# nh13/DWGSIM

Hardware: AMD Instinct MI355X
Metric: M read-pairs/sec (2x150 bp PE) (higher is better)
Workload: dtype u8

## Files before the change

dwgsim_amd/csrc/dw_host.cpp:

```cpp
#include <hip/hip_runtime.h>
#include <math.h>
#include <stdio.h>
#include <stdlib.h>
#include <string.h>
#include <limits.h>
#include <ctype.h>
#include <stdarg.h>
#include <stdint.h>
#include <sys/mman.h>
#include <mutex>
#include <thread>
#include <string>
#include <vector>
#include <algorithm>
#include <array>
#include <stddef.h>
#include <type_traits>
#include "../../include/dwgsim_hip.h"
#include "dw_kernels.hpp"
#include "dw_launch.hpp"
#include "dw_mutin.hpp"
#include "dw_mem.hpp"

using namespace dw;

namespace {

struct HostIns { std::vector<int32_t> pos; std::vector<uint32_t> len, off; std::vector<uint8_t> bases; };

struct Member {
    std::string name;
    int64_t l = 0, l_place = 0;
    uint32_t contig_index = 0;
    int32_t start = 0;
    int32_t reg_off = 0, n_reg = 0;
    uint32_t name_off = 0; int32_t name_fixed_len = 0;
    ResolvedContig rc;
};

struct GroupMem {
    DevMem d_ref, d_cells[2], d_view[2];
    DevMem d_ins_pos[2], d_ins_len[2], d_ins_off[2], d_ins_bases[2];
    DevMem d_names, d_reg, d_seg;
    std::vector<uint8_t> h_names; std::vector<int32_t> h_reg, h_seg;
    DevMem d_summ[2], d_summ2[2];
    DevMem d_refview, d_refsumm, d_refsumm2, d_dirty;
    DevEvent ev_walk, ev_walk0;
    DevMem d_hap_text[2], d_hap_rec, d_hap_pool;
    DevMem d_hap_chain[2];
    DevMem d_depth_pos, d_depth_cnt;
    HostMem h_wc;
};

struct WalkCounters {
    uint64_t unused0[7];
    uint64_t n_cand;
    uint32_t max_del;
    struct { uint32_t entries, bases; } ins[2];
    uint32_t unused1;
    uint32_t slot_over;
    uint32_t n_cand_true;
    uint64_t mut_debug[2];
    uint64_t n_listed;
    uint64_t unused2;
};
static_assert(std::is_standard_layout<WalkCounters>::value && sizeof(WalkCounters) == 16 * 8, "the walk's counter block is 16 u64 words");
static_assert(offsetof(WalkCounters, n_cand) == 7 * 8 && offsetof(WalkCounters, max_del) == 8 * 8 && offsetof(WalkCounters, ins) == 8 * 8 + 4 && offsetof(WalkCounters, slot_over) == 8 * 8 + 6 * 4 &&
              offsetof(WalkCounters, n_cand_true) == 8 * 8 + 7 * 4 && offsetof(WalkCounters, mut_debug) == 12 * 8 && offsetof(WalkCounters, n_listed) == 14 * 8, "every counter at the word the kernels were given before the block had a type");
struct WcSpan { size_t off, bytes; };
#define WC_SPAN(first, last) WcSpan{offsetof(WalkCounters, first), offsetof(WalkCounters, last) + sizeof(WalkCounters::last) - offsetof(WalkCounters, first)}
constexpr WcSpan WC_RANDOM = WC_SPAN(n_cand, n_cand_true), WC_FILE = WC_SPAN(mut_debug, mut_debug), WC_LISTED = WC_SPAN(n_listed, n_listed);

struct Group {
    bool alive = false, mutated = false, walk_pending = false;
    int first_handle = -1;
    std::vector<Member> m;
    int64_t total = 0;
    GroupMem mem;
    uint32_t n_ins[2] = {0, 0}, n_ins_bases[2] = {0, 0};
    int fixed_max = 0;
    uint32_t n_cand = 0;
    bool dirty_any = false, dirty_all = false;
    int walk_attempt = 0; uint32_t walk_cap = 0; size_t walk_cap_bases = 0; bool walk_reset = false;
    uint32_t n_patch = 0, n_patch_ev = 0;
    bool list_valid = false; std::vector<int32_t> pos; std::vector<uint32_t> cells; HostIns ins[2];
    bool depth_valid = false; std::vector<int32_t> depth_pos;
    struct HapText { bool valid = false; int width = 0; uint64_t bytes = 0; std::vector<uint64_t> off, len; std::vector<int64_t> bases; } hap_text[2];
    struct HapChain { bool valid = false; std::vector<uint64_t> first; std::vector<int64_t> ref_start; std::vector<dwgsim_hip_chain_block_t> blocks; } hap_chain[2];
};

struct HandleRef { int group = -1, k = 0; };

struct Counters {
    DevMem d; HostMem h;
    uint64_t *dev() const { return d.get<uint64_t>(); }
    uint64_t *host() const { return h.get<uint64_t>(); }
};

struct Slot {
    Counters counters;
    DevEvent ev_k0, ev_k1, ev_end, ev_done, ev_fetched;
    DevEvent ev_t0, ev_t1;
    bool pending = false, empty = true, fetch_in_flight = false;
    bool truth_timed = false;
    int group = -1;
    uint64_t n_pairs = 0, out_bytes[N_STREAMS] = {0, 0, 0, 0}, gz_bytes[N_STREAMS] = {0, 0, 0, 0};
    DevMem gz_out[N_STREAMS], gz_status, segs;
    HostMem h_segs;
    std::vector<dwgsim_hip_range_t> ranges;
    DevMem d_rerun_chain;
    int cap_mult = 1;
};

}

struct dwgsim_hip_ctx {
    dwgsim_hip_params_t prm;
    std::string read_prefix;
    struct Tables {
        std::vector<uint8_t> flow;
        DevMem d_flow;
        double e_by[2] = {0, 0};
        DevMem d_thr[2];
        DevMem d_thr32[2]; int e_full = 0;
        DevMem d_qbase[2]; int32_t qb_words = 1;
        DevMem d_rand_fixed; int32_t rand_fixed_len = 0;
    } tab;
    struct Debug {
        int site_slots = -1; int64_t site_slot_cap = -1;
        bool seq_justify = false, dense_view = false;
        int flow_cap_forced = 0;
        int ion_lds = -1;
        int flow_slots = 0;
        int64_t truth_cap = -1, truth_reruns = 0;
        int64_t walk_cap = -1, place_cap = -1; bool phases = false;
        int writer = -1, force_threads = 0, split = -1, qrows = 1;
        uint64_t place_open = 0; double walk_us = 0, count_us = 0;
        int64_t sim_form = 0;
        int64_t walk_form = 0;
        double hap_len_us = 0, hap_write_us = 0, hap_copy_us = 0, truth_us = 0, truth_copy_us = 0; bool hap_yardstick = false; double chain_count_us = 0, chain_write_us = 0; int64_t chain_blocks = 0;
    } dbg;
    int device = 0;
    DevStream stream;
    DevStream copy_stream;
    DevStream walk_stream;
    DevStream count_stream;
    std::string err;
    std::vector<Group> groups;
    std::vector<GroupMem> pool;
    std::vector<HandleRef> handles;
    DevMem meta, fail_summ, block_rand, status_all, out[DWGSIM_HIP_SLOTS][N_STREAMS], split_state, split_hand, split_agg, split_pre, split_chunk;
    DevMem w_slots, w_slot_aux;
    DevMem scratch_mask, scratch_cnt, scratch_status, w_cand, w_ev, w_flags, w_lo, w_sufmin, w_bound, w_ppos, w_pcells, up_ascii, l_pos, l_cells, place_segs, place_rand, place_list, place_aux;
    HostMem h_up; DevEvent ev_up; bool up_in_flight = false;
    HostMem h_place_segs, h_range_rand;
    std::vector<int32_t> h_ppos; std::vector<uint16_t> h_pcells; std::vector<Event> h_pev;
    MutInput mutin; bool has_mutin = false;
    Regions regions; bool has_regions = false;
    DevMem flow_scratch, flow_free;
    Counters counters;
    DevMem d_wcounters;
    Counters pcounters;
    Slot slot[DWGSIM_HIP_SLOTS];
    DevMem d_chain;
    int chain_contig = -1; uint64_t chain_next_ii = 0;
    bool has_carry_override = false; uint64_t carry_override = 0;
    int flow_cap_mult = 1;
    int n_cu = 0;
    DevEvent ev_cnt0, ev_cnt1;
    bool gzip_on = false; DevMem d_crc_table, d_crc_shift;
    bool truth_on = false;
    bool truth_md = false;
    bool depth_on = false;
    DevMem t_nl[2], t_rec[2], t_ends, t_len, t_blk;
    HostMem h_stage;
    DevStream hap_stream;
    DevEvent hap_ev[6];
    DevEvent chain_ev[4];
    int hap_cur[2] = {-1, -1};
    std::string txt, vcf;
};

namespace {

#define HIPC(ctx, call) do { hipError_t e_ = (call); if (e_ != hipSuccess) { char b_[512]; snprintf(b_, sizeof b_, "HIP error %s at %s:%d (%s)", hipGetErrorString(e_), __FILE__, __LINE__, #call); (ctx)->err = b_; return DWGSIM_HIP_ERR_DEVICE; } } while (0)

hipError_t dev_malloc(dwgsim_hip_ctx *c, void **p, size_t bytes)
{
    hipError_t e = DevKind::alloc(p, bytes);
    if (e == hipSuccess || c->pool.empty()) return e;
    (void)hipGetLastError();
    hipStreamSynchronize(c->walk_stream.get());
    c->pool.clear();
    return DevKind::alloc(p, bytes);
}

hipError_t reserve(dwgsim_hip_ctx *c, DevMem &b, size_t need, size_t want)
{
    return b.reserve(need, want, [c](void **p, size_t n) { return dev_malloc(c, p, n); });
}

int ensure(dwgsim_hip_ctx *c, DevMem &b, size_t bytes)
{
    HIPC(c, reserve(c, b, bytes, bytes + bytes / 8 + 4096));
    return 0;
}

int upload(dwgsim_hip_ctx *c, DevMem &b, const void *src, size_t n)
{
    HIPC(c, reserve(c, b, n, n));
    const hipError_t e = hipMemcpy(b.get(), src, n, hipMemcpyHostToDevice);
    if (e != hipSuccess) b.reset();
    HIPC(c, e);
    return 0;
}

template <class T> int upload_table(dwgsim_hip_ctx_t *c, DevMem &d, const std::vector<T> &h, size_t slack)
{
    HIPC(c, reserve(c, d, sizeof(T) * h.size(), sizeof(T) * (h.size() + slack)));
    HIPC(c, hipMemcpyAsync(d.get(), h.data(), sizeof(T) * h.size(), hipMemcpyHostToDevice, c->walk_stream.get()));
    return 0;
}

uint8_t nt4(int ch)
{
    switch (ch) { case 'A': case 'a': return 0; case 'C': case 'c': return 1; case 'G': case 'g': return 2; case 'T': case 't': return 3; case '-': return 5; default: return 4; }
}

void lazy_quality_params(double sigma, float *k, float *eps, float *lmin, int32_t *near1_zero)
{
    const double two_ln2 = 2.0 * log(2.0);
    double lm = 0.98 * (0.45 / sigma) * (0.45 / sigma) / two_ln2;
    if (!(lm < 0x1p-4)) lm = 0x1p-4;
    *near1_zero = lm >= 0x1p-10 ? 1 : 0;
    if (lm < 0x1p-10) lm = 0x1p-10;
    *lmin = (float)lm;
    lm = (double)*lmin * (1.0 - 0x1p-20);
    *k = (float)(sqrt(two_ln2) * sigma);
    *eps = (float)(1.5 * sigma * (3.4e-7 / sqrt(lm) + 7.2e-6) + 0x1p-18);
}

WalkParams walk_params(const dwgsim_hip_ctx *c)
{
    WalkParams w; w.mut_rate = c->prm.mut_rate; w.indel_frac = c->prm.indel_frac; w.indel_extend = c->prm.indel_extend;
    w.indel_min = c->prm.indel_min; w.is_hap = c->prm.is_hap; w.seed = (uint32_t)c->prm.seed;
    w.mut_thr = !(c->prm.mut_rate > 0) ? 0 : c->prm.mut_rate >= 1.0 ? 0x100000000ull : (uint64_t)ceil(c->prm.mut_rate * 4294967296.0);
    flow_gap_params(w.mut_thr, &w.gap_r, &w.gap_s);
    w.lg = reinterpret_cast<const uint32_t *>(c->tab.d_flow.get() + 64);
    return w;
}

size_t padded_cells(const Group &g) { return (size_t)g.total + CELL_PAD; }

size_t view_bytes(size_t padded) { return padded / 2; }
size_t summ_bytes(size_t padded) { return sizeof(uint16_t) * (padded / SUMM_CELLS); }
size_t summ2_bytes(size_t padded) { return sizeof(uint16_t) * (padded / SUMM2_CELLS); }
uint32_t dirty_words(size_t padded) { return (uint32_t)((padded + 32 * SUMM_CELLS - 1) / (32 * SUMM_CELLS)); }
size_t dirty_bytes(size_t padded) { return sizeof(uint32_t) * ((size_t)dirty_words(padded) + 2); }

enum : unsigned { R_CELLS = 1, R_VIEW = 2, R_SUMM = 4, R_SUMM2 = 8, R_ALL = 15 };
int restore_pristine(dwgsim_hip_ctx *c, const Group &g, int h, unsigned what, hipStream_t st)
{
    const GroupMem &M = g.mem;
    const size_t padded = padded_cells(g);
    if (what & R_CELLS) HIPC(c, hipMemcpyAsync(M.d_cells[h].get(), M.d_ref.get(), padded, hipMemcpyDeviceToDevice, st));
    if (what & R_VIEW) HIPC(c, hipMemcpyAsync(M.d_view[h].get(), M.d_refview.get(), view_bytes(padded), hipMemcpyDeviceToDevice, st));
    if (what & R_SUMM) HIPC(c, hipMemcpyAsync(M.d_summ[h].get(), M.d_refsumm.get(), summ_bytes(padded), hipMemcpyDeviceToDevice, st));
    if (what & R_SUMM2) HIPC(c, hipMemcpyAsync(M.d_summ2[h].get(), M.d_refsumm2.get(), summ2_bytes(padded), hipMemcpyDeviceToDevice, st));
    return 0;
}

int clear_dirty(dwgsim_hip_ctx *c, const Group &g, hipStream_t st)
{
    HIPC(c, hipMemsetAsync(g.mem.d_dirty.get(), 0, dirty_bytes(padded_cells(g)), st));
    return 0;
}

hipError_t wc_fill(dwgsim_hip_ctx *c, WcSpan s, int byte, hipStream_t st) { return hipMemsetAsync(c->d_wcounters.get() + s.off, byte, s.bytes, st); }
hipError_t wc_fetch(dwgsim_hip_ctx *c, const GroupMem &M, WcSpan s, hipStream_t st) { return hipMemcpyAsync(M.h_wc.get() + s.off, c->d_wcounters.get() + s.off, s.bytes, hipMemcpyDeviceToHost, st); }

struct InsTable { void *dev, *host; size_t bytes; };
std::array<InsTable, 4> ins_tables(const GroupMem &M, int h, HostIns &t)
{
    return {{{M.d_ins_pos[h].get(), t.pos.data(), sizeof(int32_t) * t.pos.size()}, {M.d_ins_len[h].get(), t.len.data(), sizeof(uint32_t) * t.len.size()},
             {M.d_ins_off[h].get(), t.off.data(), sizeof(uint32_t) * t.off.size()}, {M.d_ins_bases[h].get(), t.bases.data(), t.bases.size()}}};
}

SegTab seg_tab(const Group &g)
{
    const int n = (int)g.m.size();
    const int32_t *seg = g.mem.d_seg.get<int32_t>();
    SegTab t; t.start = seg; t.len = seg + (n + 1); t.cindex = reinterpret_cast<const uint32_t *>(seg + (2 * n + 1)); t.n = n;
    return t;
}

void fill_haps(const Group &g, HapDev (&hap)[2])
{
    const GroupMem &M = g.mem;
    for (int h = 0; h < 2; ++h) {
        hap[h].cells = M.d_cells[h].get(); hap[h].view = M.d_view[h].get(); hap[h].ins_pos = M.d_ins_pos[h].get<int32_t>(); hap[h].ins_len = M.d_ins_len[h].get<uint32_t>();
        hap[h].ins_off = M.d_ins_off[h].get<uint32_t>(); hap[h].ins_bases = M.d_ins_bases[h].get(); hap[h].n_ins = g.n_ins[h]; hap[h].pos_off = 0;
    }
}

ContigDev group_dev(const Group &g)
{
    ContigDev d;
    fill_haps(g, d.hap);
    d.ref = g.mem.d_ref.get(); d.l = g.total; d.seg = seg_tab(g);
    d.tot4 = nullptr; d.cap_bases[0] = d.cap_bases[1] = 0;
    return d;
}

size_t ins_bases_cap(const Group &g, int h) { const size_t cap = g.mem.d_ins_bases[h].cap(); return cap ? cap - 16 : 0; }

Group *get_group(dwgsim_hip_ctx_t *c, int contig, int *k = nullptr)
{
    if (!c) return nullptr;
    if (contig < 0 || (size_t)contig >= c->handles.size() || c->handles[(size_t)contig].group < 0) { c->err = "unknown contig handle"; return nullptr; }
    const HandleRef r = c->handles[(size_t)contig];
    Group &g = c->groups[(size_t)r.group];
    if (!g.alive) { c->err = "unknown contig handle"; return nullptr; }
    if (k) *k = r.k;
    return &g;
}

int64_t align_up(int64_t v, int64_t a) { return (v + a - 1) / a * a; }

template <class Run> int selftest_words(int device, size_t n, uint64_t *out, Run run)
{
    if (!out || hipSetDevice(device) != hipSuccess) return DWGSIM_HIP_ERR_DEVICE;
    DevMem d;
    if (d.reserve(n * sizeof(uint64_t), n * sizeof(uint64_t)) != hipSuccess) return DWGSIM_HIP_ERR_NOMEM;
    hipMemset(d.get(), 0, n * sizeof(uint64_t));
    if (const int rc = run(d.get<uint64_t>())) return rc;
    const hipError_t e = hipMemcpy(out, d.get(), n * sizeof(uint64_t), hipMemcpyDeviceToHost);
    return e == hipSuccess ? DWGSIM_HIP_OK : DWGSIM_HIP_ERR_DEVICE;
}

}

extern "C" {

void dwgsim_hip_params_default(dwgsim_hip_params_t *p)
{
    memset(p, 0, sizeof(*p));
    p->e_start[0] = p->e_end[0] = p->e_start[1] = p->e_end[1] = 0.02;
    p->dist = 500; p->std_dev = 50; p->N = -1; p->C = 100;
    p->length[0] = p->length[1] = 70;
    p->mut_rate = 0.001; p->mut_freq = 0.5; p->indel_frac = 0.1; p->indel_extend = 0.3; p->indel_min = 1;
    p->rand_read = 0.05; p->seed = -1; p->fixed_quality = -1; p->quality_std = 2.0;
}

#define CHK(v, lo, hi, nm) do { if ((v) < (lo) || (hi) < (v)) { if (msg) snprintf(msg, cap, "Error: command line option %s was out of range\n", nm); return DWGSIM_HIP_ERR_ARG; } } while (0)

int dwgsim_hip_params_check(const dwgsim_hip_params_t *p, char *msg, size_t cap)
{
    if (msg && cap) msg[0] = 0;
    CHK(p->is_inner, 0, 1, "-i"); CHK(p->dist, 0, INT32_MAX, "-d"); CHK(p->std_dev, 0, INT32_MAX, "-s");
    if (p->N < 0 && p->C < 0) { if (msg) snprintf(msg, cap, "Must use one of -N or -C"); return DWGSIM_HIP_ERR_ARG; }
    else if (0 < p->N && 0 < p->C) { if (msg) snprintf(msg, cap, "Cannot use both -N or -C"); return DWGSIM_HIP_ERR_ARG; }
    else if (0 < p->N) { CHK(p->N, 1, INT32_MAX, "-N"); CHK(p->C, INT32_MIN, -1, "-C"); }
    else { CHK(p->N, INT32_MIN, -1, "-N"); CHK(p->C, 0, INT32_MAX, "-C"); }
    CHK(p->length[0], 1, INT32_MAX, "-1"); CHK(p->length[1], 0, INT32_MAX, "-2");
    for (int i = 0; i < 2; ++i) {
        if (p->e_start[i] < 0.0 || 1.0 < p->e_start[i]) { if (msg) snprintf(msg, cap, "End %s: the start error is out of range (-e)\n", i ? "two" : "one"); return DWGSIM_HIP_ERR_ARG; }
        if (p->e_end[i] < 0.0 || 1.0 < p->e_end[i]) { if (msg) snprintf(msg, cap, "End %s: the end error is out of range (-e)\n", i ? "two" : "one"); return DWGSIM_HIP_ERR_ARG; }
        if (p->data_type == 2 && p->e_end[i] != p->e_start[i]) { if (msg) snprintf(msg, cap, "End %s: a uniform error rate must be given for Ion Torrent data\n", i ? "two" : "one"); return DWGSIM_HIP_ERR_ARG; }
    }
    CHK(p->mut_rate, 0, 1.0, "-r"); CHK(p->indel_frac, 0, 1.0, "-R"); CHK(p->indel_extend, 0, 1.0, "-X");
    CHK(p->indel_min, 1, INT32_MAX, "-I"); CHK(p->data_type, 0, 2, "-c"); CHK(p->strandedness, 0, 2, "-S");
    CHK(p->read_one_strand, 0, 2, "-A"); CHK(p->max_n, 0, INT32_MAX, "-n"); CHK(p->rand_read, 0, 1.0, "-y");
    if (p->data_type == 2 && !p->flow_order) { if (msg) snprintf(msg, cap, "Error: command line option -f is required\n"); return DWGSIM_HIP_ERR_ARG; }
    CHK(p->use_base_error, 0, 1, "-B"); CHK(p->is_hap, 0, 1, "-H");
    if (p->fixed_quality < -1 || p->fixed_quality > 255) { if (msg) snprintf(msg, cap, "Error: command line option -q requires one character\n"); return DWGSIM_HIP_ERR_ARG; }
    CHK(p->quality_std, 0, INT32_MAX, "-Q"); CHK(p->reads_output_type, 0, 2, "-o");
    CHK(p->output_type, 0, 2, "-M"); CHK(p->amplicons, 0, 1, "-a");
    if (p->data_type == 2) {
        const size_t F = strlen(p->flow_order);
        bool has[4] = {false, false, false, false};
        for (size_t i = 0; i < F; ++i) { const uint8_t c = nt4((unsigned char)p->flow_order[i]); if (c < 4) has[c] = true; }
        bool only_acgt = true; for (size_t i = 0; i < F; ++i) if (nt4((unsigned char)p->flow_order[i]) >= 4) only_acgt = false;
        if (F == 0 || F > 64 || !only_acgt || !(has[0] && has[1] && has[2] && has[3])) { if (msg) snprintf(msg, cap, "dwgsim-hip: the flow order (-f) must hold 1..64 flows and contain all of A, C, G, T\n"); return DWGSIM_HIP_ERR_UNSUP; }
    }
    if (p->seed < 0) { if (msg) snprintf(msg, cap, "dwgsim-hip: the seed must be resolved (>= 0) before the context is created\n"); return DWGSIM_HIP_ERR_ARG; }
    return DWGSIM_HIP_OK;
}

int64_t dwgsim_hip_pairs_for_contig(const dwgsim_hip_params_t *p, int64_t l, uint64_t tot_len, int is_last_contig, int64_t n_sim_so_far)
{
    int64_t n_pairs = 0;
    const int size0 = p->length[0], size1 = p->length[1];
    if (is_last_contig && p->C < 0) n_pairs = p->N - n_sim_so_far;
    else if (0 < p->N) {
        n_pairs = (int64_t)(uint64_t)((long double)l / tot_len * p->N + 0.5);
        if (p->N - n_sim_so_far < n_pairs) n_pairs = p->N - n_sim_so_far;
    } else n_pairs = (int64_t)(uint64_t)(l * p->C / ((long double)(size0 + size1)) / (1.0 - p->rand_read) + 0.5);
    const int max_len = size0 > size1 ? size0 : size1;
    if (p->amplicons == 1) { if (l < max_len) return DWGSIM_HIP_SKIP_AMPLICON; }
    else if (0 < size1 && l < p->dist + 3 * p->std_dev) return DWGSIM_HIP_SKIP_SHORT_INSERT;
    else if (l < size0 || (0 < size1 && l < size1)) return DWGSIM_HIP_SKIP_SHORT_READ;
    return n_pairs < 0 ? DWGSIM_HIP_SKIP_NO_PAIRS : n_pairs;
}

int dwgsim_hip_device_numa_node(int device)
{
    char bus[64] = {0};
    if (hipDeviceGetPCIBusId(bus, (int)sizeof bus, device) != hipSuccess) { (void)hipGetLastError(); return -1; }
    for (char *q = bus; *q; ++q) *q = (char)tolower((unsigned char)*q);
    char path[160]; snprintf(path, sizeof path, "/sys/bus/pci/devices/%s/numa_node", bus);
    FILE *f = fopen(path, "r");
    if (!f) return -1;
    int node = -1;
    if (fscanf(f, "%d", &node) != 1) node = -1;
    fclose(f);
    return node;
}

int dwgsim_hip_device_info(int device, char *name, size_t cap, int *n_cu, size_t *hbm_bytes)
{
    hipDeviceProp_t pr;
    if (hipGetDeviceProperties(&pr, device) != hipSuccess) return DWGSIM_HIP_ERR_DEVICE;
    if (name && cap) snprintf(name, cap, "%s (%s)", pr.name, pr.gcnArchName);
    if (n_cu) *n_cu = pr.multiProcessorCount;
    if (hbm_bytes) *hbm_bytes = pr.totalGlobalMem;
    return DWGSIM_HIP_ABI_VERSION;
}

// ... 396 lines not shown
        for (size_t q = 0; q < c->regions.contig.size(); ++q) if (c->regions.contig[q] == m.contig_index) { st.push_back((int32_t)c->regions.start[q]); en.push_back((int32_t)c->regions.end[q]); tot += c->regions.end[q] - c->regions.start[q]; }
        m.reg_off = (int32_t)M.h_reg.size(); m.n_reg = (int32_t)st.size(); m.l_place = tot;
        M.h_reg.insert(M.h_reg.end(), st.begin(), st.end()); M.h_reg.insert(M.h_reg.end(), en.begin(), en.end());
    }
    M.h_reg.push_back(0);
    return upload_table(c, M.d_reg, M.h_reg, 64);
}

static int build_group(dwgsim_hip_ctx_t *c, Group &g, const uint8_t *const *ascii, const int64_t *lens, const int64_t *starts)
{
    const int n = (int)g.m.size();
    const size_t padded = padded_cells(g);
    bool must_wait = true;
    if (const int rc = reserve_cell_buffers(c, g.mem, padded)) return rc;
    if (const int rc = upload_sequence(c, n, ascii, lens, starts, g.total, padded, must_wait)) return rc;
    if (const int rc = make_pristine(c, g)) return rc;
    if (const int rc = upload_group_tables(c, g)) return rc;
    if (c->has_mutin) for (int k = 0; k < n; ++k) resolve_mutation_input(c->mutin, g.m[(size_t)k].contig_index, ascii[k], lens[k], (uint32_t)c->prm.seed, c->prm.is_hap != 0, g.m[(size_t)k].rc);
    if (must_wait) HIPC(c, hipStreamSynchronize(c->walk_stream.get()));
    return 0;
}

int dwgsim_hip_add_contigs(dwgsim_hip_ctx_t *c, int n, const char *const *names, const uint8_t *const *ascii, const int64_t *lens, const uint32_t *contig_index)
{
    if (!c || n < 1 || !names || !ascii || !lens || !contig_index) { if (c) c->err = "bad contig arguments"; return DWGSIM_HIP_ERR_ARG; }
    for (int k = 0; k < n; ++k) if (!names[k] || (!ascii[k] && lens[k] > 0) || lens[k] < 0 || lens[k] > INT32_MAX) { c->err = "bad contig arguments"; return DWGSIM_HIP_ERR_ARG; }
    std::vector<int64_t> starts((size_t)n);
    const int64_t total = dwgsim_hip_group_layout(lens, n, starts.data());
    if (total < 0 || total > (int64_t)INT32_MAX - 2 * GROUP_ALIGN) { c->err = "dwgsim-hip: the contigs of one group must stay below 2^31 cells in all (add them in smaller groups)\n"; return DWGSIM_HIP_ERR_ARG; }
    HIPC(c, hipSetDevice(c->device));
    const int gid = take_group(c, (size_t)total + CELL_PAD);
    Group &g = c->groups[(size_t)gid];
    g.alive = true; g.total = total; g.first_handle = (int)c->handles.size();
    g.m.resize((size_t)n);
    for (int k = 0; k < n; ++k) { Member &m = g.m[(size_t)k]; m.name = names[k]; m.l = m.l_place = lens[k]; m.contig_index = contig_index[k]; m.start = (int32_t)starts[(size_t)k]; }
    const int rc = build_group(c, g, ascii, lens, starts.data());
    if (rc != 0) { (void)hipStreamSynchronize(c->walk_stream.get()); g = Group(); return rc; }
    for (int k = 0; k < n; ++k) c->handles.push_back(HandleRef{gid, k});
    return g.first_handle;
}

int dwgsim_hip_add_contig(dwgsim_hip_ctx_t *c, const char *name, const uint8_t *ascii, int64_t len, uint32_t contig_index)
{
    return dwgsim_hip_add_contigs(c, 1, &name, &ascii, &len, &contig_index);
}

int dwgsim_hip_drop_contig(dwgsim_hip_ctx_t *c, int contig)
{
    Group *g = get_group(c, contig);
    if (!g) return DWGSIM_HIP_ERR_ARG;
    hipSetDevice(c->device);
    const int gid = (int)(g - c->groups.data());
    for (int s = 0; s < DWGSIM_HIP_SLOTS; ++s) if (c->slot[s].pending && !c->slot[s].empty && c->slot[s].group == gid) { c->err = "drop_contig: a batch that reads this group has not been waited for (dwgsim_hip_wait first)"; return DWGSIM_HIP_ERR_STATE; }
    if (g->walk_pending) hipEventSynchronize(g->mem.ev_walk.get());
    for (size_t k = 0; k < g->m.size(); ++k) { if (c->chain_contig == g->first_handle + (int)k) c->chain_contig = -1; c->handles[(size_t)g->first_handle + k].group = -1; }
    for (int h = 0; h < 2; ++h) if (c->hap_cur[h] == gid) c->hap_cur[h] = -1;
    c->pool.push_back(std::move(g->mem));
    *g = Group();
    if (c->pool.size() > 3) {
        hipStreamSynchronize(c->walk_stream.get());
        c->pool.erase(c->pool.begin());
    }
    return DWGSIM_HIP_OK;
}

int dwgsim_hip_set_regions(dwgsim_hip_ctx_t *c, const char *path, const char *const *names, const int64_t *lens, int n_contigs, uint64_t *total_len)
{
    if (!c || !path || n_contigs < 0 || (n_contigs && (!names || !lens))) { if (c) c->err = "bad regions arguments"; return DWGSIM_HIP_ERR_ARG; }
    if (c->prm.amplicons) { c->err = "Error: cannot use a regions BED file (-x) when simulating amplicons (-a)\n"; return DWGSIM_HIP_ERR_ARG; }
    std::vector<ContigName> tab;
    for (int i = 0; i < n_contigs; ++i) tab.push_back(ContigName{names[i], lens[i]});
    std::string err;
    if (!parse_regions(path, tab, c->regions, err)) { c->err = err; c->has_regions = false; return DWGSIM_HIP_ERR_ARG; }
    c->has_regions = true;
    uint64_t tot = 0;
    for (size_t q = 0; q < c->regions.start.size(); ++q) tot += c->regions.end[q] - c->regions.start[q];
    if (total_len) *total_len = tot;
    return DWGSIM_HIP_OK;
}

int64_t dwgsim_hip_contig_region_length(dwgsim_hip_ctx_t *c, uint32_t contig_index, const uint8_t *ascii, int64_t len, int64_t *non_acgt, int64_t *region_bases)
{
    if (non_acgt) *non_acgt = 0;
    if (region_bases) *region_bases = len;
    if (!c || !c->has_regions) return len;
    int64_t m = 0, num_n = 0;
    for (size_t q = 0; q < c->regions.contig.size(); ++q) if (c->regions.contig[q] == contig_index) {
        m += c->regions.end[q] - c->regions.start[q];
        for (int64_t p = c->regions.start[q]; p <= (int64_t)c->regions.end[q]; ++p) { const int ch = (p >= 1 && p - 1 < len) ? ascii[p - 1] : 'N'; if (nt4(ch) >= 4) ++num_n; }
    }
    if (non_acgt) *non_acgt = num_n;
    if (region_bases) *region_bases = m;
    if (m == 0) return DWGSIM_HIP_SKIP_NO_REGION;
    if (0.95 < num_n / (double)m) return DWGSIM_HIP_SKIP_NON_ACGT;
    return m;
}

int dwgsim_hip_contig_set_placement_length(dwgsim_hip_ctx_t *c, int contig, int64_t l)
{
    int k = 0;
    Group *g = get_group(c, contig, &k);
    if (!g || l < 0) { if (c) c->err = "bad placement-length arguments"; return DWGSIM_HIP_ERR_ARG; }
    g->m[(size_t)k].l_place = l;
    return DWGSIM_HIP_OK;
}

int dwgsim_hip_set_mutation_input(dwgsim_hip_ctx_t *c, int type, const char *path, const char *const *names, const int64_t *lens, int n_contigs)
{
    if (!c || !path || type < 0 || type > 2 || n_contigs < 0 || (n_contigs && (!names || !lens))) { if (c) c->err = "bad mutation-input arguments"; return DWGSIM_HIP_ERR_ARG; }
    std::vector<ContigName> tab;
    for (int i = 0; i < n_contigs; ++i) tab.push_back(ContigName{names[i], lens[i]});
    std::string err;
    if (!parse_mutation_input(type, path, tab, c->mutin, err)) { c->err = err; c->has_mutin = false; return DWGSIM_HIP_ERR_ARG; }
    c->has_mutin = true;
    return DWGSIM_HIP_OK;
}

static int mut_debug_verdict(dwgsim_hip_ctx_t *c, const Group &g, uint64_t pre, uint64_t post)
{
    auto member_of = [&](uint64_t v) -> int { const int64_t p = (int64_t)(v >> 8); int k = 0; while (k + 1 < (int)g.m.size() && (int64_t)g.m[(size_t)k + 1].start <= p) ++k; return k; };
    uint64_t v = ~0ull;
    if (pre != ~0ull && post != ~0ull) v = member_of(post) < member_of(pre) ? post : pre;
    else v = pre != ~0ull ? pre : post;
    if (v == ~0ull) return DWGSIM_HIP_OK;
    static const char *what[4] = {"", "(c[0]&0x3) != (c[1]&0x3)", "(c[1]&0x3) != (c[2]&0x3)", "(c[0]&0x3) == (c[1]&0x3) || (c[0]&0x3) == (c[2]&0x3)"};
    const Member &m = g.m[(size_t)member_of(v)];
    char b[256]; snprintf(b, sizeof b, "dwgsim: src/mut.c: mut_debug: Assertion `%s' failed. [%s:%lld]\n", what[v & 3], m.name.c_str(), (long long)(v >> 8) - m.start + 1);
    c->err = b;
    return DWGSIM_HIP_ERR_FAILED;
}

static int ensure_ins(dwgsim_hip_ctx_t *c, Group &g, int h, size_t entries, size_t bases)
{
    GroupMem &M = g.mem;
    const size_t want = sizeof(int32_t) * (entries + entries / 4 + 64);
    for (DevMem *b : {&M.d_ins_pos[h], &M.d_ins_len[h], &M.d_ins_off[h]}) HIPC(c, reserve(c, *b, sizeof(int32_t) * entries, want));
    HIPC(c, reserve(c, M.d_ins_bases[h], bases + 16, bases + bases / 4 + 256 + 16));
    return DWGSIM_HIP_OK;
}

static void make_views(hipStream_t st, const Group &g)
{
    const GroupMem &M = g.mem;
    launch_make_view(st, M.d_cells[0].get(), M.d_cells[1].get(), (int64_t)padded_cells(g) & ~(int64_t)15, g.total, M.d_view[0].get(), M.d_view[1].get(),
                     M.d_summ[0].get<uint16_t>(), M.d_summ[1].get<uint16_t>(), M.d_summ2[0].get<uint16_t>(), M.d_summ2[1].get<uint16_t>());
}

static void dirty_chunks(hipStream_t st, bool restore, const Group &g)
{
    const GroupMem &M = g.mem;
    launch_dirty_chunks(st, restore, M.d_dirty.get<uint32_t>(), dirty_words(padded_cells(g)), g.total, M.d_ref.get(), M.d_refview.get(), M.d_refsumm.get<uint16_t>(), M.d_refsumm2.get<uint16_t>(),
                        M.d_cells[0].get(), M.d_cells[1].get(), M.d_view[0].get(), M.d_view[1].get(), M.d_summ[0].get<uint16_t>(), M.d_summ[1].get<uint16_t>(), M.d_summ2[0].get<uint16_t>(), M.d_summ2[1].get<uint16_t>());
}

static void justify(dwgsim_hip_ctx_t *c, hipStream_t st, const Event *ev, Count n, const ContigDev &cd)
{
    if (c->dbg.seq_justify) launch_justify_seq(st, ev, n, cd);
    else launch_justify(st, ev, n, cd, c->w_lo.get<int32_t>(), c->w_sufmin.get<int32_t>(), c->w_bound.get<uint8_t>());
}

static int64_t pack_walk_form(int attempt, bool file_driven, bool slots, int restore, bool dense)
{
    return (int64_t)attempt << 16 | (file_driven ? 1 : 0) << 12 | (slots ? 1 : 0) << 8 | restore << 4 | (dense ? 1 : 0);
}

static int walk_file_driven(dwgsim_hip_ctx_t *c, Group &g)
{
    hipStream_t st = c->walk_stream.get();
    const GroupMem &M = g.mem;
    WalkCounters *wc = c->d_wcounters.get<WalkCounters>();
    const uint32_t np = g.n_patch, nev = g.n_patch_ev;
    const size_t nev1 = nev ? nev : 1;
    if (np && (ensure(c, c->w_ppos, sizeof(int32_t) * np) || ensure(c, c->w_pcells, sizeof(uint16_t) * np) || ensure(c, c->w_ev, sizeof(Event) * nev1) ||
               ensure(c, c->w_lo, sizeof(int32_t) * nev1) || ensure(c, c->w_sufmin, sizeof(int32_t) * (nev1 + 64)) || ensure(c, c->w_bound, nev1))) return DWGSIM_HIP_ERR_DEVICE;
    c->dbg.walk_form = pack_walk_form(g.walk_attempt, true, false, g.walk_reset ? 2 : 0, true);
    HIPC(c, hipEventRecord(M.ev_walk0.get(), st));
    if (g.walk_reset) for (int h = 0; h < 2; ++h) if (const int rc = restore_pristine(c, g, h, R_CELLS, st)) return rc;
    HIPC(c, wc_fill(c, WC_FILE, 0xff, st));
    if (np) {
        HIPC(c, hipMemcpyAsync(c->w_ppos.get(), c->h_ppos.data(), sizeof(int32_t) * np, hipMemcpyHostToDevice, st));
        HIPC(c, hipMemcpyAsync(c->w_pcells.get(), c->h_pcells.data(), sizeof(uint16_t) * np, hipMemcpyHostToDevice, st));
        if (nev) HIPC(c, hipMemcpyAsync(c->w_ev.get(), c->h_pev.data(), sizeof(Event) * nev, hipMemcpyHostToDevice, st));
        launch_apply_patches(st, c->w_ppos.get<int32_t>(), c->w_pcells.get<uint16_t>(), np, M.d_cells[0].get(), M.d_cells[1].get());
        launch_mut_debug(st, M.d_ref.get(), M.d_cells[0].get(), M.d_cells[1].get(), g.total, &wc->mut_debug[0]);
        if (nev) justify(c, st, c->w_ev.get<Event>(), Count{nullptr, nev}, group_dev(g));
        launch_mut_debug(st, M.d_ref.get(), M.d_cells[0].get(), M.d_cells[1].get(), g.total, &wc->mut_debug[1]);
    }
    make_views(st, g);
    g.dirty_all = true;
    HIPC(c, hipGetLastError());
    HIPC(c, wc_fetch(c, M, WC_FILE, st));
    HIPC(c, hipEventRecord(M.ev_walk.get(), st));
    return DWGSIM_HIP_OK;
}

enum class Restore { None, Chunks, All };
struct WalkPlan {
    uint32_t cap; size_t ncap, cap_bases;
    uint32_t nblk;
    bool use_slots; uint32_t nbs, slot_cap; size_t slot_bytes;
    Restore restore;
    bool dense;
};

static WalkPlan walk_plan(const dwgsim_hip_ctx_t *c, const Group &g)
{
    WalkPlan P;
    P.cap = g.walk_cap; P.ncap = P.cap ? P.cap : 1; P.cap_bases = g.walk_cap_bases;
    P.nblk = (uint32_t)((g.total + SCAN_POS_PER_BLOCK - 1) / SCAN_POS_PER_BLOCK);
    P.nbs = site_scan_blocks(g.total);
    const double m = (double)site_scan_block_positions() * (c->prm.mut_rate > 0 ? c->prm.mut_rate : 0.0);
    P.slot_cap = (uint32_t)std::min<double>((double)site_scan_block_positions(), m + 8.0 * sqrt(m + 1.0) + 32.0);
    if (c->dbg.site_slot_cap >= 0) P.slot_cap = (uint32_t)std::max<int64_t>(1, c->dbg.site_slot_cap);
    P.slot_bytes = (size_t)P.nbs * P.slot_cap * sizeof(int32_t);
    P.use_slots = g.walk_attempt == 0 && c->dbg.site_slots != 0 && P.nbs > 0 && (c->dbg.site_slots > 0 || P.slot_bytes <= std::max<size_t>((size_t)64 << 20, P.ncap * 16));
    P.restore = g.walk_attempt > 0 || g.dirty_all ? Restore::All : g.dirty_any ? Restore::Chunks : Restore::None;
    P.dense = c->dbg.seq_justify || c->dbg.dense_view;
    return P;
}

static int walk_reserve(dwgsim_hip_ctx_t *c, Group &g, const WalkPlan &P)
{
    if (ensure(c, c->scratch_status, ((size_t)P.nblk + 2) * sizeof(uint64_t)) ||
        ensure(c, c->w_cand, sizeof(int32_t) * P.ncap) || ensure(c, c->w_ev, sizeof(Event) * P.ncap) ||
        ensure(c, c->w_flags, sizeof(uint4) * (P.ncap + 64)) ||
        ensure(c, c->w_lo, sizeof(int32_t) * P.ncap) || ensure(c, c->w_sufmin, sizeof(int32_t) * (P.ncap + 64)) ||
        ensure(c, c->w_bound, P.ncap)) return DWGSIM_HIP_ERR_DEVICE;
    for (int h = 0; h < 2; ++h) if (const int rc = ensure_ins(c, g, h, P.ncap, P.cap_bases)) return rc;
    if (P.use_slots && (ensure(c, c->w_slots, P.slot_bytes) || ensure(c, c->w_slot_aux, 2 * (size_t)P.nbs * sizeof(uint32_t)))) return DWGSIM_HIP_ERR_DEVICE;
    return DWGSIM_HIP_OK;
}

static int walk_launch(dwgsim_hip_ctx_t *c, Group &g, const WalkPlan &P)
{
    hipStream_t st = c->walk_stream.get();
    const WalkParams wp = walk_params(c);
    const SegTab seg = seg_tab(g);
    const GroupMem &M = g.mem;
    WalkCounters *wc = c->d_wcounters.get<WalkCounters>();
    int32_t *d_cand = c->w_cand.get<int32_t>(); Event *d_ev = c->w_ev.get<Event>(); uint4 *d_flags = c->w_flags.get<uint4>();
    uint32_t *tot4 = &wc->ins[0].entries;
    const Count nc{&wc->n_cand, P.cap};
    HIPC(c, wc_fill(c, WC_RANDOM, 0, st));
    if (P.use_slots) launch_site_scan_slots(st, M.d_refview.get(), g.total, seg, wp, c->w_slots.get<int32_t>(), P.slot_cap, c->w_slot_aux.get<uint32_t>(), d_cand, P.cap, &wc->n_cand, &wc->slot_over);
    else {
        uint64_t *d_status = c->scratch_status.get<uint64_t>();
        HIPC(c, hipMemsetAsync(d_status, 0, ((size_t)P.nblk + 2) * sizeof(uint64_t), st));
        launch_site_scan_list(st, M.d_refview.get(), g.total, seg, wp, d_status, d_status + P.nblk, d_cand, P.cap, &wc->n_cand);
    }
    launch_events(st, d_cand, nc, M.d_ref.get(), seg, wp, d_ev, &wc->max_del);
    launch_resolve(st, d_ev, nc, &wc->max_del, d_flags, tot4);
    ContigDev cd = group_dev(g);
    cd.tot4 = tot4; cd.cap_bases[0] = (uint32_t)std::min<size_t>(ins_bases_cap(g, 0), 0xFFFFFFFFu); cd.cap_bases[1] = (uint32_t)std::min<size_t>(ins_bases_cap(g, 1), 0xFFFFFFFFu);
    launch_apply(st, d_ev, nc, d_flags, cd, wp);
    justify(c, st, d_ev, nc, cd);
    if (P.dense) {
        make_views(st, g);
        g.dirty_all = true;
    } else {
        launch_mark_dirty(st, d_ev, nc, c->w_lo.get<int32_t>(), M.d_dirty.get<uint32_t>());
        dirty_chunks(st, false, g);
        g.dirty_any = true;
    }
    HIPC(c, hipGetLastError());
    return DWGSIM_HIP_OK;
}

static int walk_random(dwgsim_hip_ctx_t *c, Group &g)
{
    const WalkPlan P = walk_plan(c, g);
    if (const int rc = walk_reserve(c, g, P)) return rc;
    c->dbg.walk_form = pack_walk_form(g.walk_attempt, false, P.use_slots, (int)P.restore, P.dense);
    hipStream_t st = c->walk_stream.get();
    HIPC(c, hipEventRecord(g.mem.ev_walk0.get(), st));
    if (P.restore == Restore::All) { for (int h = 0; h < 2; ++h) if (const int rc = restore_pristine(c, g, h, R_ALL, st)) return rc; }
    else if (P.restore == Restore::Chunks) dirty_chunks(st, true, g);
    if (P.restore != Restore::None) { if (const int rc = clear_dirty(c, g, st)) return rc; g.dirty_all = g.dirty_any = false; }
    if (const int rc = walk_launch(c, g, P)) return rc;
    HIPC(c, wc_fetch(c, g.mem, WC_RANDOM, st));
    HIPC(c, hipEventRecord(g.mem.ev_walk.get(), st));
    return DWGSIM_HIP_OK;
}

static void collect_file_mutations(dwgsim_hip_ctx_t *c, const Group &g, HostIns (&hi)[2])
{
    c->h_ppos.clear(); c->h_pcells.clear(); c->h_pev.clear();
    for (size_t k = 0; k < g.m.size(); ++k) {
        const Member &m = g.m[k];
        for (size_t q = 0; q < m.rc.pos.size(); ++q) {
            c->h_ppos.push_back(m.rc.pos[q] + m.start); c->h_pcells.push_back(m.rc.cells[q]);
            if (m.rc.cells[q] & 0x3030) { Event e; e.pos = m.rc.pos[q] + m.start; e.type = 4; e.hap = 3; e.base = 0; e.live = 1; e.len = 1; e.seg = (uint32_t)k; c->h_pev.push_back(e); }
        }
        for (int h = 0; h < 2; ++h) for (const InsPayload &ip : m.rc.ins[h]) {
            hi[h].pos.push_back(ip.pos + m.start); hi[h].len.push_back((uint32_t)ip.bases.size()); hi[h].off.push_back((uint32_t)hi[h].bases.size());
            hi[h].bases.insert(hi[h].bases.end(), ip.bases.begin(), ip.bases.end());
        }
    }
}

static int upload_ins_tables(dwgsim_hip_ctx_t *c, Group &g, HostIns (&hi)[2])
{
    for (int h = 0; h < 2; ++h) {
        const size_t n = hi[h].pos.size(), nb = hi[h].bases.size();
        g.n_ins[h] = (uint32_t)n; g.n_ins_bases[h] = (uint32_t)nb;
        if (const int rc = ensure_ins(c, g, h, n ? n : 1, nb ? nb : 1)) return rc;
        if (n) for (const InsTable &t : ins_tables(g.mem, h, hi[h])) HIPC(c, hipMemcpy(t.dev, t.host, t.bytes, hipMemcpyHostToDevice));
    }
    return DWGSIM_HIP_OK;
}

static void initial_walk_caps(const dwgsim_hip_ctx_t *c, Group &g)
{
    double mean = 0;
    for (const Member &m : g.m) mean += (double)m.l * c->prm.mut_rate;
    g.walk_cap = (uint32_t)std::min<double>((double)g.total, mean + 8.0 * sqrt(mean + 1.0) + 256.0);
    g.walk_cap_bases = (size_t)g.walk_cap * 8 + 4096;
    if (c->dbg.walk_cap >= 0) { g.walk_cap = (uint32_t)c->dbg.walk_cap; g.walk_cap_bases = 1; }
}

int dwgsim_hip_mutate_async(dwgsim_hip_ctx_t *c, int contig)
{
    Group *gp = get_group(c, contig);
    if (!gp) return DWGSIM_HIP_ERR_ARG;
    Group &g = *gp;
    if (g.walk_pending) { c->err = "mutate: the group's previous walk was not waited for"; return DWGSIM_HIP_ERR_STATE; }
    for (const Slot &sl : c->slot) if (sl.pending && sl.group == c->handles[(size_t)contig].group) { c->err = "mutate: a batch that reads this group is still in flight (wait for it first)"; return DWGSIM_HIP_ERR_STATE; }
    HIPC(c, hipSetDevice(c->device));
    g.walk_reset = g.mutated;
    for (int h = 0; h < 2; ++h) g.n_ins[h] = g.n_ins_bases[h] = 0;
    g.mutated = true; g.n_cand = 0; g.list_valid = false; g.depth_valid = false;
    for (int h = 0; h < 2; ++h) g.hap_text[h].valid = g.hap_chain[h].valid = false;
    g.walk_attempt = 0;
    if (g.total == 0) return DWGSIM_HIP_OK;
    if (c->has_mutin) {
        HIPC(c, hipStreamSynchronize(c->walk_stream.get()));
        HostIns hi[2];
        collect_file_mutations(c, g, hi);
        g.n_patch = (uint32_t)c->h_ppos.size(); g.n_patch_ev = (uint32_t)c->h_pev.size();
        g.n_cand = g.n_patch_ev;
        HIPC(c, hipStreamSynchronize(c->walk_stream.get()));
        if (const int rc = upload_ins_tables(c, g, hi)) return rc;
    } else initial_walk_caps(c, g);
    if (const int rc = c->has_mutin ? walk_file_driven(c, g) : walk_random(c, g)) return rc;
    g.walk_pending = true;
    return DWGSIM_HIP_OK;
}

static bool walk_fits(const WalkCounters &w, const Group &g)
{
    return !w.slot_over && w.n_cand <= g.walk_cap && w.ins[0].bases <= ins_bases_cap(g, 0) && w.ins[1].bases <= ins_bases_cap(g, 1);
}

static void exact_walk_caps(const WalkCounters &w, Group &g)
{
    g.walk_cap = (uint32_t)std::min<uint64_t>((uint64_t)g.total, (w.slot_over ? (uint64_t)w.n_cand_true : w.n_cand) + 16);
    g.walk_cap_bases = std::max<size_t>(g.walk_cap_bases, (size_t)std::max(w.ins[0].bases, w.ins[1].bases) * 2 + (size_t)g.walk_cap * 8 + 4096);
}

int dwgsim_hip_mutate_wait(dwgsim_hip_ctx_t *c, int contig)
{
    Group *gp = get_group(c, contig);
    if (!gp) return DWGSIM_HIP_ERR_ARG;
    Group &g = *gp;
    if (!g.walk_pending) return g.mutated ? DWGSIM_HIP_OK : (c->err = "mutate_wait: no walk was enqueued for this group", DWGSIM_HIP_ERR_STATE);
    HIPC(c, hipSetDevice(c->device));
    const WalkCounters &w = *g.mem.h_wc.get<WalkCounters>();
    for (;;) {
        HIPC(c, hipEventSynchronize(g.mem.ev_walk.get()));
        { float ms = 0; if (hipEventElapsedTime(&ms, g.mem.ev_walk0.get(), g.mem.ev_walk.get()) == hipSuccess) c->dbg.walk_us += 1e3 * ms; else (void)hipGetLastError(); }
        if (c->has_mutin) {
            g.walk_pending = false;
            return g.n_patch ? mut_debug_verdict(c, g, w.mut_debug[0], w.mut_debug[1]) : DWGSIM_HIP_OK;
        }
        const bool fits = walk_fits(w, g);
        if (fits || g.walk_attempt >= 2) {
            g.walk_pending = false;
            if (!fits) { c->err = "mutation walk: capacities still exceeded after an exact re-run"; return DWGSIM_HIP_ERR_FAILED; }
            g.n_cand = (uint32_t)w.n_cand;
            for (int h = 0; h < 2; ++h) { g.n_ins[h] = w.ins[h].entries; g.n_ins_bases[h] = w.ins[h].bases; }
            return DWGSIM_HIP_OK;
        }
        exact_walk_caps(w, g);
        ++g.walk_attempt;
        if (const int rc = walk_random(c, g)) { g.walk_pending = false; return rc; }
    }
}

int dwgsim_hip_mutate_poll(dwgsim_hip_ctx_t *c, int contig)
{
    Group *gp = get_group(c, contig);
    if (!gp) return DWGSIM_HIP_ERR_ARG;
    if (!gp->walk_pending) return 1;
    HIPC(c, hipSetDevice(c->device));
    const hipError_t e = hipEventQuery(gp->mem.ev_walk.get());
    if (e == hipSuccess) return 1;
    (void)hipGetLastError();
    return e == hipErrorNotReady ? 0 : (c->err = "mutate_poll: device error", DWGSIM_HIP_ERR_DEVICE);
}

int dwgsim_hip_mutate_contig(dwgsim_hip_ctx_t *c, int contig)
{
    const int rc = dwgsim_hip_mutate_async(c, contig);
    if (rc != DWGSIM_HIP_OK) return rc;
    return dwgsim_hip_mutate_wait(c, contig);
}

namespace {
struct TextOut {
    std::string &s;
    void ch(char c) { s.push_back(c); }
    void str(const char *p, size_t n) { s.append(p, n); }
    void lit(const char *p) { s.append(p); }
    void num(long long v)
    {
        char b[24]; int n = 0; unsigned long long u = v < 0 ? 0ull - (unsigned long long)v : (unsigned long long)v;
        do { b[n++] = (char)('0' + u % 10); u /= 10; } while (u);
        if (v < 0) s.push_back('-');
        while (n) s.push_back(b[--n]);
    }
};
struct ListView {
    const int32_t *pos; const uint32_t *cells; size_t n; const HostIns *ins;
};
void ins_text(const HostIns &t, int32_t pos, std::string &tmp)
{
    tmp.clear();
    auto it = std::lower_bound(t.pos.begin(), t.pos.end(), pos);
    if (it == t.pos.end() || *it != pos) return;
    const size_t k = (size_t)(it - t.pos.begin());
    for (uint32_t q = 0; q < t.len[k]; ++q) tmp.push_back("ACGTN"[t.bases[t.off[k] + q] & 3]);
}
void format_mutations(const ListView &g, const std::string &name, int64_t s0, int64_t l, std::string &txt_s, std::string &vcf_s, const uint64_t *depth = nullptr, std::string *tvcf_s = nullptr)
{
    txt_s.clear(); vcf_s.clear();
    if (tvcf_s) tvcf_s->clear();
    const size_t e0 = (size_t)(std::lower_bound(g.pos, g.pos + g.n, (int32_t)s0) - g.pos);
    const size_t e1 = (size_t)(std::lower_bound(g.pos, g.pos + g.n, (int32_t)(s0 + l)) - g.pos);
    txt_s.reserve((e1 - e0) * (name.size() + 20)); vcf_s.reserve((e1 - e0) * (name.size() + 56));
    static const char B5[] = "ACGTN";
    TextOut txt{txt_s}, vcf{vcf_s};
    std::string tmp;
    auto cell = [&](size_t e, int h) -> uint8_t { return (uint8_t)(h ? g.cells[e] >> 8 : g.cells[e]); };
    auto refc = [&](size_t e) -> uint8_t { return (uint8_t)(g.cells[e] >> 16); };
    auto prevc = [&](size_t e) -> uint8_t { return (uint8_t)(g.cells[e] >> 24); };
    size_t rec_at = 0;
    auto vcf_head = [&](long long at) { rec_at = vcf_s.size(); vcf.str(name.data(), name.size()); vcf.ch('\t'); vcf.num(at); vcf.lit("\t.\t"); };
    auto sample = [&](size_t e, int pl) {
        if (!tvcf_s) return;
        TextOut t{*tvcf_s};
        t.str(vcf_s.data() + rec_at, vcf_s.size() - rec_at - 1);
        const uint64_t n1 = depth ? depth[2 * (e - e0)] : 0, n2 = depth ? depth[2 * (e - e0) + 1] : 0;
        const uint64_t alt = pl == 3 ? n1 + n2 : pl == 1 ? n1 : n2;
        const uint64_t ref = pl == 3 ? 0 : (cell(e, pl == 1 ? 1 : 0) & TMASK) == T_NONE ? (pl == 1 ? n2 : n1) : 0;
        t.lit("\tGT:AD:DP\t"); t.lit(pl == 3 ? "1|1" : pl == 1 ? "1|0" : "0|1");
        t.ch(':'); t.num((long long)ref); t.ch(','); t.num((long long)alt); t.ch(':'); t.num((long long)(n1 + n2)); t.ch('\n');
    };
    for (size_t e = e0; e < e1; ++e) {
        const int64_t i = g.pos[e] - s0;
        const uint8_t r0 = refc(e), c1 = cell(e, 0), c2 = cell(e, 1);
        if (r0 >= 4) continue;
        const bool adj = e > e0 && g.pos[e - 1] == g.pos[e] - 1;
        const bool prev0 = adj && (cell(e - 1, 0) & TMASK) != T_NONE, prev1 = adj && (cell(e - 1, 1) & TMASK) != T_NONE;
        txt.str(name.data(), name.size()); txt.ch('\t'); txt.num((long long)i + 1); txt.ch('\t');
        const bool hom = (c1 & BTMASK) == (c2 & BTMASK);
        const uint8_t t1 = c1 & TMASK, t2 = c2 & TMASK;
        if (hom ? t1 == T_SUB : (t1 == T_SUB || t2 == T_SUB)) {
            if (hom) {
                txt.ch(B5[r0]); txt.ch('\t'); txt.ch(B5[c1 & 0xf]); txt.lit("\t3\n");
                vcf_head((long long)i + 1); vcf.ch(B5[r0]); vcf.ch('\t'); vcf.ch(B5[c1 & 0xf]); vcf.lit("\t100\tPASS\tAF=1.0;pl=3;mt=SUBSTITUTE\n");
                sample(e, 3);
            } else {
                const int hap = t1 == T_SUB ? 1 : 2;
                txt.ch(B5[r0]); txt.ch('\t'); txt.ch("XACMGRSVTWYHKDBN"[1 << (c1 & 3) | 1 << (c2 & 3)]); txt.ch('\t'); txt.ch((char)('0' + hap)); txt.ch('\n');
                vcf_head((long long)i + 1); vcf.ch(B5[r0]); vcf.ch('\t'); vcf.ch(B5[(hap == 1 ? c1 : c2) & 0xf]); vcf.lit("\t100\tPASS\tAF=0.5;pl="); vcf.ch((char)('0' + hap)); vcf.lit(";mt=SUBSTITUTE\n");
                sample(e, hap);
            }
        } else if (hom ? t1 == T_DEL : (t1 == T_DEL || t2 == T_DEL)) {
            const int pl = hom ? 3 : (t1 == T_DEL ? 1 : 2);
            txt.ch(B5[r0]); txt.lit("\t-\t"); txt.ch((char)('0' + pl)); txt.ch('\n');
            const bool open = hom ? (!prev0 || !prev1) : !(pl == 1 ? prev0 : prev1);
            if (open) {
                vcf_head((long long)i);
                if (i > 0) vcf.ch(B5[prevc(e)]);
                size_t ee = e; int64_t j = i;
                for (;;) {
                    vcf.ch(B5[refc(ee)]);
                    if (j + 1 >= l) break;
                    if (ee + 1 < e1 && g.pos[ee + 1] - s0 == j + 1) {
                        ++ee; ++j;
                        const uint8_t a1 = cell(ee, 0), a2 = cell(ee, 1);
                        const bool h2 = (a1 & BTMASK) == (a2 & BTMASK);
                        if (!(h2 == hom && ((pl == 2 ? a2 : a1) & TMASK) == T_DEL)) break;
                    } else break;
                }
                if (i > 0) { vcf.ch('\t'); vcf.ch(B5[prevc(e)]); } else vcf.lit("\t.");
                vcf.lit("\t100\tPASS\tAF="); vcf.lit(hom ? "1.0" : "0.5"); vcf.lit(";pl="); vcf.ch((char)('0' + pl)); vcf.lit(";mt=DELETE\n");
                sample(e, pl);
            }
        } else {
            const int pl = hom ? 3 : (t1 == T_INS ? 1 : 2);
            ins_text(g.ins[pl == 2 ? 1 : 0], g.pos[e], tmp);
            txt.lit("-\t"); txt.str(tmp.data(), tmp.size()); txt.ch('\t'); txt.ch((char)('0' + pl)); txt.ch('\n');
            vcf_head((long long)i + 1); vcf.ch(B5[r0]); vcf.ch('\t'); vcf.ch(B5[r0]); vcf.str(tmp.data(), tmp.size());
            vcf.lit("\t100\tPASS\tAF="); vcf.lit(hom ? "1.0" : "0.5"); vcf.lit(";pl="); vcf.ch((char)('0' + pl)); vcf.lit(";mt=INSERT\n");
            sample(e, pl);
        }
    }
}

int collect_listed_positions(dwgsim_hip_ctx_t *c, Group &g, uint32_t *n_out)
{
    *n_out = 0;
    if (g.total <= 0 || g.n_cand == 0) return DWGSIM_HIP_OK;
    hipStream_t st = c->walk_stream.get();
    const uint32_t nblk = (uint32_t)((g.total + SCAN_POS_PER_BLOCK - 1) / SCAN_POS_PER_BLOCK);
    if (ensure(c, c->scratch_mask, (size_t)nblk * SCAN_THREADS * sizeof(uint16_t))) return DWGSIM_HIP_ERR_DEVICE;
    if (ensure(c, c->scratch_cnt, (size_t)nblk * sizeof(uint32_t))) return DWGSIM_HIP_ERR_DEVICE;
    uint16_t *d_mask = c->scratch_mask.get<uint16_t>(); uint32_t *d_cnt = c->scratch_cnt.get<uint32_t>();
    launch_collect_mask(st, g.mem.d_cells[0].get(), g.mem.d_cells[1].get(), g.total, d_mask, d_cnt);
    launch_scan_excl(st, d_cnt, nblk, &c->d_wcounters.get<WalkCounters>()->n_listed);
    HIPC(c, wc_fetch(c, g.mem, WC_LISTED, st));
    HIPC(c, hipStreamSynchronize(st));
    const uint32_t n = (uint32_t)g.mem.h_wc.get<WalkCounters>()->n_listed;
    if (n) {
        if (ensure(c, c->l_pos, sizeof(int32_t) * (size_t)n)) return DWGSIM_HIP_ERR_DEVICE;
        launch_compact(st, d_mask, d_cnt, c->l_pos.get<int32_t>(), g.total, n);
    }
    *n_out = n;
    return DWGSIM_HIP_OK;
}
// ... 922 lines not shown
    return DWGSIM_HIP_OK;
}

int dwgsim_hip_set_truth_depth(dwgsim_hip_ctx_t *c, int on)
{
    if (!c) return DWGSIM_HIP_ERR_ARG;
    for (const Slot &sl : c->slot) if (sl.pending) { c->err = "set_truth_depth: a batch is in flight (wait for every slot first)"; return DWGSIM_HIP_ERR_STATE; }
    if (on && c->prm.data_type != 0) {
        c->err = c->prm.data_type == 1 ? "dwgsim-hip: no true read depth for SOLiD reads (-c 1): it is counted from the alignments of the truth SAM, which colour space does not have\n"
                                       : "dwgsim-hip: no true read depth for Ion Torrent reads (-c 2): it is counted from the alignments of the truth SAM, which the flow model's own indels rule out\n";
        return DWGSIM_HIP_ERR_UNSUP;
    }
    if (on) { HIPC(c, hipSetDevice(c->device)); for (Slot &sl : c->slot) { HIPC(c, sl.ev_t0.create()); HIPC(c, sl.ev_t1.create()); } }
    c->depth_on = on != 0;
    return DWGSIM_HIP_OK;
}
int64_t dwgsim_hip_truth_depth_fetch(dwgsim_hip_ctx_t *c, int contig, uint64_t *counts, size_t cap_cells)
{
    int km = 0;
    Group *gp = c ? get_group(c, contig, &km) : nullptr;
    if (!gp) return DWGSIM_HIP_ERR_ARG;
    if (!c->depth_on) { c->err = "truth_depth_fetch: the true read depth is switched off (dwgsim_hip_set_truth_depth)"; return DWGSIM_HIP_ERR_ARG; }
    if (!counts && cap_cells) { c->err = "bad truth_depth_fetch arguments"; return DWGSIM_HIP_ERR_ARG; }
    Group &g = *gp;
    if (!g.mutated || g.walk_pending) { c->err = "mutate_contig must run first"; return DWGSIM_HIP_ERR_STATE; }
    HIPC(c, hipSetDevice(c->device));
    if (const int rc = depth_prepare(c, g)) return rc;
    const Member &m = g.m[(size_t)km];
    const auto b = g.depth_pos.begin(), e = g.depth_pos.end();
    const size_t e0 = (size_t)(std::lower_bound(b, e, m.start) - b), e1 = (size_t)(std::lower_bound(b, e, (int32_t)(m.start + m.l)) - b);
    const size_t n = e1 - e0, take = n < cap_cells ? n : cap_cells;
    if (take) HIPC(c, hipMemcpyAsync(counts, g.mem.d_depth_cnt.get<uint64_t>() + 2 * e0, 2 * sizeof(uint64_t) * take, hipMemcpyDeviceToHost, c->stream.get()));
    HIPC(c, hipStreamSynchronize(c->stream.get()));
    return (int64_t)n;
}

int64_t dwgsim_hip_truth_vcf_header(const char *const *names, const int64_t *lens, int n, char *buf, size_t cap)
{
    if (n < 0 || (n > 0 && (!names || !lens)) || (!buf && cap)) return DWGSIM_HIP_ERR_ARG;
    std::string h = "##fileformat=VCFv4.1\n";
    for (int k = 0; k < n; ++k) { if (!names[k]) return DWGSIM_HIP_ERR_ARG; h += "##contig=<ID="; h += names[k]; h += ",length=" + std::to_string((int)lens[k]) + ">\n"; }
    h += "##INFO=<ID=AF,Number=A,Type=Float,Description=\"Allele Frequency\">\n"
         "##INFO=<ID=pl,Number=1,Type=Integer,Description=\"Phasing: 1 - HET contig 1, #2 - HET contig #2, 3 - HOM both contigs\">\n"
         "##INFO=<ID=mt,Number=1,Type=String,Description=\"Variant Type: SUBSTITUTE/INSERT/DELETE\">\n"
         "##FORMAT=<ID=GT,Number=1,Type=String,Description=\"Genotype, phased: haplotype 1 | haplotype 2\">\n"
         "##FORMAT=<ID=AD,Number=.,Type=Integer,Description=\"Simulated read ends that hold the site, by the haplotype they were read from: ref,alt\">\n"
         "##FORMAT=<ID=DP,Number=1,Type=Integer,Description=\"Simulated read ends that hold the site, both haplotypes\">\n"
         "#CHROM\tPOS\tID\tREF\tALT\tQUAL\tFILTER\tINFO\tFORMAT\tdwgsim\n";
    if (buf) memcpy(buf, h.data(), h.size() < cap ? h.size() : cap);
    return (int64_t)h.size();
}

int64_t dwgsim_hip_truth_sam_header(const char *const *names, const int64_t *lens, int n, char *buf, size_t cap)
{
    if (n < 0 || (n > 0 && (!names || !lens)) || (!buf && cap)) return DWGSIM_HIP_ERR_ARG;
    std::string h = "@HD\tVN:1.6\tSO:unsorted\tGO:query\n";
    for (int k = 0; k < n; ++k) { if (!names[k]) return DWGSIM_HIP_ERR_ARG; h += "@SQ\tSN:"; h += names[k]; h += "\tLN:" + std::to_string((long long)lens[k]) + "\n"; }
    h += "@PG\tID:dwgsim-hip\tPN:dwgsim-hip\tDS:true alignments of the simulated reads\n";
    if (buf) memcpy(buf, h.data(), h.size() < cap ? h.size() : cap);
    return (int64_t)h.size();
}

int dwgsim_hip_fetch_wait(dwgsim_hip_ctx_t *c, int slot)
{
    if (!c || slot < 0 || slot >= DWGSIM_HIP_SLOTS) { if (c) c->err = "bad slot"; return DWGSIM_HIP_ERR_ARG; }
    Slot &sl = c->slot[slot];
    if (!sl.fetch_in_flight) return DWGSIM_HIP_OK;
    HIPC(c, hipSetDevice(c->device));
    HIPC(c, hipEventSynchronize(sl.ev_fetched.get()));
    sl.fetch_in_flight = false;
    return DWGSIM_HIP_OK;
}

int dwgsim_hip_fetch(dwgsim_hip_ctx_t *c, int slot, int stream, void *host_dst, size_t cap)
{
    if (!is_slot_stream(c, slot, stream) || (!host_dst && cap)) return DWGSIM_HIP_ERR_ARG;
    HIPC(c, hipSetDevice(c->device));
    Slot &sl = c->slot[slot];
    if (sl.pending) { c->err = "fetch: wait for the batch first (its sizes are not known yet)"; return DWGSIM_HIP_ERR_STATE; }
    const size_t n = (size_t)sl.out_bytes[stream];
    if (n > cap) { c->err = "fetch: destination too small"; return DWGSIM_HIP_ERR_ARG; }
    if (n == 0) return DWGSIM_HIP_OK;
    if (is_page_locked(host_dst)) {
        HIPC(c, hipMemcpyAsync(host_dst, c->out[slot][stream].get(), n, hipMemcpyDeviceToHost, c->copy_stream.get()));
        HIPC(c, hipStreamSynchronize(c->copy_stream.get()));
        return DWGSIM_HIP_OK;
    }
    const size_t CH = (size_t)16 << 20;
    HIPC(c, c->h_stage.reserve(2 * CH, 2 * CH));
    const uint8_t *src = c->out[slot][stream].get<uint8_t>();
    uint8_t *stage[2] = {c->h_stage.get<uint8_t>(), c->h_stage.get<uint8_t>() + CH};
    size_t done = 0; int b = 0;
    size_t cur = n < CH ? n : CH;
    HIPC(c, hipMemcpyAsync(stage[0], src, cur, hipMemcpyDeviceToHost, c->copy_stream.get()));
    while (done < n) {
        HIPC(c, hipStreamSynchronize(c->copy_stream.get()));
        const size_t next_off = done + cur, next = next_off < n ? ((n - next_off) < CH ? (n - next_off) : CH) : 0;
        if (next) HIPC(c, hipMemcpyAsync(stage[b ^ 1], src + next_off, next, hipMemcpyDeviceToHost, c->copy_stream.get()));
        memcpy((uint8_t *)host_dst + done, stage[b], cur);
        done += cur; cur = next; b ^= 1;
    }
    return DWGSIM_HIP_OK;
}

int dwgsim_hip_debug_count_byte(dwgsim_hip_ctx_t *c, int slot, int stream, int byte, uint64_t *count)
{
    if (!is_slot_stream(c, slot, stream) || !count) return DWGSIM_HIP_ERR_ARG;
    HIPC(c, hipSetDevice(c->device));
    Slot &sl = c->slot[slot];
    if (sl.pending) { c->err = "count_byte: wait for the batch first"; return DWGSIM_HIP_ERR_STATE; }
    HIPC(c, hipMemsetAsync(&c->counters.dev()[COUNT_BYTE_COUNTER], 0, sizeof(uint64_t), c->stream.get()));
    if (sl.out_bytes[stream]) launch_count_byte(c->stream.get(), c->out[slot][stream].get<uint8_t>(), sl.out_bytes[stream], (uint32_t)(byte & 0xff), &c->counters.dev()[COUNT_BYTE_COUNTER]);
    HIPC(c, hipMemcpyAsync(&c->counters.host()[COUNT_BYTE_COUNTER], &c->counters.dev()[COUNT_BYTE_COUNTER], sizeof(uint64_t), hipMemcpyDeviceToHost, c->stream.get()));
    HIPC(c, hipStreamSynchronize(c->stream.get()));
    *count = c->counters.host()[COUNT_BYTE_COUNTER];
    return DWGSIM_HIP_OK;
}

int dwgsim_hip_debug_gzip(dwgsim_hip_ctx_t *c, const void *text, size_t n, void *out, size_t cap, size_t *out_n)
{
    if (!c || (!text && n) || !out_n) return DWGSIM_HIP_ERR_ARG;
    HIPC(c, hipSetDevice(c->device));
    if (const int rc = dwgsim_hip_set_gzip(c, c->gzip_on ? 1 : 0); rc < 0) return rc;
    if (!c->d_crc_shift) { const bool was = c->gzip_on; if (const int rc = dwgsim_hip_set_gzip(c, 1); rc < 0) return rc; c->gzip_on = was; }
    *out_n = 0;
    if (n == 0) return DWGSIM_HIP_OK;
    const size_t gcap = (size_t)gz_capacity(n), nch = (size_t)gz_chunks(n);
    DevMem text_m, out_m, aux_m;
    if (reserve(c, text_m, n + 64, n + 64) != hipSuccess || reserve(c, out_m, gcap + 64, gcap + 64) != hipSuccess || reserve(c, aux_m, sizeof(uint64_t) * (4 + nch), sizeof(uint64_t) * (4 + nch)) != hipSuccess) { c->err = "out of device memory"; return DWGSIM_HIP_ERR_DEVICE; }
    uint8_t *d_text = text_m.get(), *d_out = out_m.get(); uint64_t *d_aux = aux_m.get<uint64_t>();
    const uint64_t n64 = n;
    bool ok = hipMemcpyAsync(d_text, text, n, hipMemcpyHostToDevice, c->stream.get()) == hipSuccess && hipMemsetAsync(d_aux, 0, sizeof(uint64_t) * (4 + nch), c->stream.get()) == hipSuccess &&
              hipMemcpyAsync(d_aux, &n64, sizeof n64, hipMemcpyHostToDevice, c->stream.get()) == hipSuccess;
    if (ok) {
        launch_gzip(c->stream.get(), d_text, &d_aux[0], n, d_out, gcap, &d_aux[4], &d_aux[1], &d_aux[2], &d_aux[3], c->d_crc_table.get<uint32_t>(), c->d_crc_shift.get<uint32_t>());
        uint64_t res[4] = {0, 0, 0, 0};
        ok = hipGetLastError() == hipSuccess && hipMemcpyAsync(res, d_aux, sizeof res, hipMemcpyDeviceToHost, c->stream.get()) == hipSuccess && hipStreamSynchronize(c->stream.get()) == hipSuccess;
        if (ok && (res[3] & GZIP_ROOM_BIT)) { c->err = "dwgsim-hip: the gzip output buffer is too small for this text\n"; return DWGSIM_HIP_ERR_FAILED; }
        if (ok && res[2] > cap) { c->err = "debug_gzip: destination too small"; return DWGSIM_HIP_ERR_ARG; }
        if (ok) { ok = hipMemcpy(out, d_out, (size_t)res[2], hipMemcpyDeviceToHost) == hipSuccess; *out_n = (size_t)res[2]; }
    }
    if (!ok) { c->err = "debug_gzip: device error"; return DWGSIM_HIP_ERR_DEVICE; }
    return DWGSIM_HIP_OK;
}

int dwgsim_hip_debug_option(dwgsim_hip_ctx_t *c, const char *key, int64_t value)
{
    if (!c || !key) return DWGSIM_HIP_ERR_ARG;
    if (!strcmp(key, "justify_seq")) c->dbg.seq_justify = value != 0;
    else if (!strcmp(key, "dense_view")) c->dbg.dense_view = value != 0;
    else if (!strcmp(key, "walk_cap")) c->dbg.walk_cap = value;
    else if (!strcmp(key, "site_slots")) c->dbg.site_slots = (int)value;
    else if (!strcmp(key, "site_slot_cap")) c->dbg.site_slot_cap = value;
    else if (!strcmp(key, "phases")) c->dbg.phases = value != 0;
    else if (!strcmp(key, "writer")) c->dbg.writer = (int)value;
    else if (!strcmp(key, "sim_threads")) c->dbg.force_threads = (int)value;
    else if (!strcmp(key, "walk_seg_min")) walk_debug_seg_min((uint32_t)value);
    else if (!strcmp(key, "place_cap")) c->dbg.place_cap = value;
    else if (!strcmp(key, "truth_cap")) c->dbg.truth_cap = value;
    else if (!strcmp(key, "split")) c->dbg.split = (int)value;
    else if (!strcmp(key, "qrows")) c->dbg.qrows = (int)value;
    else if (!strcmp(key, "flow_slots")) c->dbg.flow_slots = (int)value;
    else if (!strcmp(key, "ion_lds")) c->dbg.ion_lds = (int)value;
    else if (!strcmp(key, "flow_cap")) c->dbg.flow_cap_forced = (int)value;
    else if (!strcmp(key, "hap_yardstick")) c->dbg.hap_yardstick = value != 0;
    else if (!strcmp(key, "truth_yardstick")) {
        Slot &sl = c->slot[0];
        if (!c->truth_on || sl.pending || value <= 0 || (uint64_t)value > sl.out_bytes[3]) { c->err = "truth_yardstick: slot 0 holds no truth SAM of that size"; return DWGSIM_HIP_ERR_ARG; }
        HIPC(c, hipSetDevice(c->device));
        DevMem tmp;
        HIPC(c, reserve(c, tmp, (size_t)value, (size_t)value));
        HIPC(c, hipEventRecord(sl.ev_t0.get(), c->stream.get()));
        HIPC(c, hipMemcpyAsync(tmp.get(), c->out[0][3].get(), (size_t)value, hipMemcpyDeviceToDevice, c->stream.get()));
        HIPC(c, hipEventRecord(sl.ev_t1.get(), c->stream.get()));
        HIPC(c, hipStreamSynchronize(c->stream.get()));
        float ms = 0; HIPC(c, hipEventElapsedTime(&ms, sl.ev_t0.get(), sl.ev_t1.get()));
        c->dbg.truth_copy_us = 1e3 * ms;
    }
    else { c->err = "unknown debug option"; return DWGSIM_HIP_ERR_ARG; }
    return DWGSIM_HIP_OK;
}

int dwgsim_hip_debug_get(dwgsim_hip_ctx_t *c, const char *key, int64_t *value)
{
    if (!c || !key || !value) return DWGSIM_HIP_ERR_ARG;
    if (!strcmp(key, "place_open")) *value = (int64_t)c->dbg.place_open;
    else if (!strcmp(key, "flow_cap_mult")) *value = (int64_t)c->flow_cap_mult;
    else if (!strcmp(key, "walk_us")) *value = (int64_t)c->dbg.walk_us;
    else if (!strcmp(key, "count_us")) *value = (int64_t)c->dbg.count_us;
    else if (!strcmp(key, "sim_form")) *value = c->dbg.sim_form;
    else if (!strcmp(key, "hap_len_us")) *value = (int64_t)c->dbg.hap_len_us;
    else if (!strcmp(key, "hap_write_us")) *value = (int64_t)c->dbg.hap_write_us;
    else if (!strcmp(key, "hap_copy_us")) *value = (int64_t)c->dbg.hap_copy_us;
    else if (!strcmp(key, "chain_count_us")) *value = (int64_t)c->dbg.chain_count_us;
    else if (!strcmp(key, "chain_write_us")) *value = (int64_t)c->dbg.chain_write_us;
    else if (!strcmp(key, "chain_blocks")) *value = c->dbg.chain_blocks;
    else if (!strcmp(key, "truth_us")) *value = (int64_t)c->dbg.truth_us;
    else if (!strcmp(key, "truth_reruns")) *value = c->dbg.truth_reruns;
    else if (!strcmp(key, "truth_copy_us")) *value = (int64_t)c->dbg.truth_copy_us;
    else if (!strcmp(key, "walk_form")) *value = c->dbg.walk_form;
    else { c->err = "unknown debug value"; return DWGSIM_HIP_ERR_ARG; }
    return DWGSIM_HIP_OK;
}

int dwgsim_hip_debug_sim_instances(int64_t *out, int cap)
{
    return sim_instances(out, cap);
}

}
```

dwgsim_amd/csrc/dw_kernels.hpp:

```cpp
#pragma once
#include <stdint.h>

namespace dw {

constexpr int PAIRS_PER_BLOCK = 128;
constexpr int PLACE_PAIRS = 256;
constexpr int PLACE_LISTS = 64;
#ifndef DW_SIM_THREADS
#define DW_SIM_THREADS 256
#endif
constexpr int SIM_THREADS = DW_SIM_THREADS;
constexpr int FLOW_STACK_WORDS = 4;
constexpr uint32_t FLOW_NEVER = 0xFFFFFFFFu;
constexpr int FLOW_LG_ENTRIES = 257;
constexpr int FLOW_CAP_MAX = 1 << 20;
constexpr int FLOW_STACK_WORDS_MAX = 32;
#ifndef DW_ION_THREADS_SMALL
#define DW_ION_THREADS_SMALL 128
#endif
constexpr int ION_THREADS_SMALL = DW_ION_THREADS_SMALL;
constexpr int SIM_THREADS_LONG = 64;
constexpr int SIM_FIFO_BYTES = 40;
constexpr int SIM_FIFO_BYTES_WIDE = 72;
inline size_t sim_lds_bytes(size_t words_per_lane, size_t lanes, size_t qb_words, bool fifo, size_t fifo_bytes = SIM_FIFO_BYTES) { return ((words_per_lane * lanes + 2 * qb_words + 3) & ~(size_t)3) * 4 + (fifo ? lanes * fifo_bytes : 0); }
inline int sim_blocks_per_cu(size_t dyn_lds, int cap) { const size_t per = (dyn_lds + 1700 + 1279) / 1280 * 1280;       const int b = (int)(163840 / per); return b < cap ? b : cap; }
constexpr size_t SIM_LDS_BUDGET = 150 * 1024;
struct SimForm {
    int lpp, out, dt, nthr, wr, split;
    size_t lds, lds_b;
    int cap, lds_words, stack_words;
};
constexpr int SCAN_POS_PER_THREAD = 16;
constexpr int SCAN_THREADS = 256;
constexpr int SCAN_POS_PER_BLOCK = SCAN_POS_PER_THREAD * SCAN_THREADS;
constexpr int CELL_PAD = 64;
constexpr int GROUP_ALIGN = SCAN_POS_PER_BLOCK;
constexpr int MAX_ATTEMPTS = 10000;

constexpr uint8_t T_NONE = 0x00, T_INS = 0x10, T_SUB = 0x20, T_DEL = 0x30, TMASK = 0x30, BTMASK = 0x3f;

struct Event {
    int32_t  pos;
    uint8_t  type;
    uint8_t  hap;
    uint8_t  base;
    uint8_t  live;
    uint32_t len;
    uint32_t seg;
};

struct SegTab { const int32_t *start; const int32_t *len; const uint32_t *cindex; int32_t n; };

struct HapDev {
    uint8_t *cells;
    const uint8_t *view;
    int32_t *ins_pos;
    uint32_t *ins_len;
    uint32_t *ins_off;
    uint8_t *ins_bases;
    uint32_t n_ins;
    int32_t pos_off;
};

struct ContigDev {
    HapDev hap[2];
    const uint8_t *ref;
    int64_t l;
    SegTab seg;
    const uint32_t *tot4;
    uint32_t cap_bases[2];
};

struct HapRec { uint64_t rec_off; uint32_t hdr_off, hdr_len, base0, n_bases; uint32_t pad_; };
struct ChainEnt { uint32_t pos, info; };
constexpr uint32_t CHAIN_END = 0x80000000u;
constexpr int HAP_WINDOW = 8192;

struct Count { const uint64_t *dev; uint32_t host; };

struct WalkParams {
    double mut_rate, indel_frac, indel_extend;
    uint64_t mut_thr;
    uint64_t gap_r; int32_t gap_s;
    const uint32_t *lg;
    int32_t indel_min, is_hap;
    uint32_t seed;
};

struct SimParams {
    double std_dev, mut_freq, rand_read, quality_std;
    int32_t dist, is_inner, len[2], max_n, strandedness, read_one_strand, amplicons, fixed_quality, data_type;
    int32_t has_bwa, has_bfast;
    uint32_t seed;
    float q_k, q_eps, q_lmin; int32_t q_near1;
};

inline uint64_t flow_ilog2_fixed(uint64_t y, int fb)
{
    const int p = 63 - __builtin_clzll(y);
    uint64_t m = y << (63 - p), frac = 0;
    for (int k = 0; k < fb; ++k) {
        const unsigned __int128 sq = (unsigned __int128)m * m;
        if ((uint64_t)(sq >> 127)) { m = (uint64_t)(sq >> 64); frac = (frac << 1) | 1u; }
        else { m = (uint64_t)(sq >> 63); frac <<= 1; }
    }
    return ((uint64_t)p << fb) | frac;
}
inline void flow_log2_table(uint32_t *lg)
{
    for (int i = 0; i < 256; ++i) lg[i] = (uint32_t)flow_ilog2_fixed(256u + (uint64_t)i, 32);
    lg[256] = 0xFFFFFFFFu;
}
inline void flow_gap_params(uint64_t thr, uint64_t *R, int32_t *s)
{
    *R = 0; *s = 0;
    if (thr == 0 || thr >= 0x100000000ull) return;
    const uint64_t Lq = (32ull << 56) - flow_ilog2_fixed(0x100000000ull - thr, 56);
    const int sh = __builtin_clzll(Lq);
    const unsigned __int128 q = ((unsigned __int128)1 << 127) / (Lq << sh);
    if ((uint64_t)(q >> 64)) { *R = 1ull << 63; *s = 62 - sh; }
    else { *R = (uint64_t)q; *s = 63 - sh; }
}

struct CalibArgs {
    uint32_t seed; int32_t end, len; uint64_t n_reads, first_read, chunk_reads;
    uint64_t thr;
    uint64_t gap_r; int32_t gap_s;
    const uint8_t *flow; int32_t flow_len, lds_words, stack_words;
    uint32_t *scratch;
    uint64_t *counters;
};

constexpr int SUMM_CELLS = 64;
constexpr int SUMM2_CELLS = 1024;

inline constexpr int flow_words_per_lane(int lds_words) { return lds_words | 1; }

struct SimSeg {
    uint32_t first_block;
    uint32_t contig_index;
    int32_t  start, l;
    uint64_t first_ii, n_pairs;
    uint64_t pair_off;
    int64_t  l_place;
    int32_t  reg_off, n_reg;
    uint32_t name_off; int32_t name_fixed_len;
    uint32_t contig_start;
    uint32_t pad_;
};

constexpr int N_COUNTERS = 32;
constexpr int N_STREAMS = 4;
constexpr int N_PHASES = 8;
constexpr int STATUS_COUNTER = 2;
constexpr int TICKET_COUNTER = 0;
constexpr int RETRY_COUNTER = 1;
constexpr int RANDOM_COUNTER = 3;
constexpr int text_len_counter(int t) { return t < 3 ? 4 + t : 7; }
constexpr int phase_counter(int k) { return 8 + k; }
constexpr int fail_seg_counter(int q) { return 16 + q; }
constexpr int ABORT_COUNTER = 20;
constexpr int CARRY_COUNTER = 21;
constexpr int CHAIN_BASE_COUNTER = 22;
constexpr int TRUTH_FIT_COUNTER = 23;
constexpr int gz_len_counter(int t) { return 24 + t; }
constexpr int gz_ticket_counter(int t) { return 28 + t; }
constexpr int gz_src_len_counter(int t, bool truth_md) { return t == 3 && truth_md ? TRUTH_FIT_COUNTER : text_len_counter(t); }
constexpr int PLACE_OPEN_COUNTER = 5;
constexpr int CALIB_ERR_COUNTER = 8;
constexpr int CALIB_LEN_COUNTER = 9;
constexpr int COUNT_BYTE_COUNTER = 15;
constexpr unsigned long long ATTEMPTS_BIT = 1;
constexpr unsigned long long FLOW_ROOM_BIT = 2;
constexpr unsigned long long REGIONS_BIT = 4;
constexpr unsigned long long GZIP_ROOM_BIT = 8;
constexpr unsigned long long PLACE_ROOM_BIT = 16;
constexpr unsigned long long TRUTH_ERR_BIT = 32;
constexpr unsigned long long TRUTH_ROOM_BIT = 64;
constexpr bool counter_claim(uint32_t &seen, int w) { if (w < 0 || w >= N_COUNTERS || (seen >> w & 1u)) return false; seen |= 1u << w; return true; }
constexpr bool slot_counters_ok()
{
    uint32_t seen = 0;
    bool ok = counter_claim(seen, TICKET_COUNTER) && counter_claim(seen, RETRY_COUNTER) && counter_claim(seen, STATUS_COUNTER) && counter_claim(seen, RANDOM_COUNTER) && counter_claim(seen, ABORT_COUNTER) &&
              counter_claim(seen, CARRY_COUNTER) && counter_claim(seen, CHAIN_BASE_COUNTER) && counter_claim(seen, TRUTH_FIT_COUNTER);
    for (int k = 0; k < N_PHASES; ++k) ok = ok && counter_claim(seen, phase_counter(k));
    for (int q = 0; q < 4; ++q) ok = ok && counter_claim(seen, fail_seg_counter(q));
    for (int t = 0; t < N_STREAMS; ++t) ok = ok && counter_claim(seen, text_len_counter(t)) && counter_claim(seen, gz_len_counter(t)) && counter_claim(seen, gz_ticket_counter(t));
    return ok;
}
constexpr bool place_counters_ok() { uint32_t seen = 0; return counter_claim(seen, RETRY_COUNTER) && counter_claim(seen, STATUS_COUNTER) && counter_claim(seen, RANDOM_COUNTER) && counter_claim(seen, PLACE_OPEN_COUNTER); }
constexpr bool context_counters_ok() { uint32_t seen = 0; return counter_claim(seen, STATUS_COUNTER) && counter_claim(seen, CALIB_ERR_COUNTER) && counter_claim(seen, CALIB_LEN_COUNTER) && counter_claim(seen, COUNT_BYTE_COUNTER); }
static_assert(slot_counters_ok(), "slot block: two words collide or one lies behind N_COUNTERS");
static_assert(place_counters_ok(), "place block: two words collide or one lies behind N_COUNTERS");
static_assert(context_counters_ok(), "context block: two words collide or one lies behind N_COUNTERS");

struct SimArgs {
    SimParams p;
    HapDev hap[2];
    const SimSeg *segs; int32_t n_seg; uint32_t n_blocks;
    uint64_t n_pairs;
    const uint64_t *chain;
    const int32_t *reg; int32_t have_regions;
    const uint64_t *e_thr[2];
    const uint16_t *summ[2];
    const uint16_t *summ2[2];
    int32_t place_fast, place_k;
    uint32_t *place_list, *place_list_n; uint32_t place_list_cap;
    uint64_t *range_rand;
    const uint32_t *e_thr32[2];
    int32_t e_full;
    const uint32_t *qbase[2];
    int32_t qb_words;
    const uint8_t *names;
    const uint8_t *rand_fixed; int32_t rand_fixed_len;
    uint32_t *meta;
    uint32_t *block_rand;
    uint64_t *counters;
    uint64_t *status[4];
    uint8_t *out[3];
    int32_t lds_words;
    int32_t cap;
    int32_t ion_lds;
    int32_t flow_stack_words;
    int32_t fifo;
    int32_t sim_threads;
    int32_t flow_len;
    int32_t split;
    uint32_t *split_state;
    uint32_t *split_hand;
    uint32_t *split_agg;
    uint64_t *split_pre;
// ... 27 lines not shown
```

dwgsim_amd/csrc/dw_launch.hpp:

```cpp
#pragma once
#include <hip/hip_runtime.h>
#include "dw_kernels.hpp"

namespace dw {
void launch_pack(hipStream_t st, const uint8_t *ascii, uint8_t *ref, uint8_t *h0, uint8_t *h1, int64_t l);
void launch_site_scan_list(hipStream_t st, const uint8_t *refview, int64_t l, SegTab seg, WalkParams wp, uint64_t *status, uint64_t *ticket, int32_t *out, uint32_t cap, uint64_t *n_out);
uint32_t site_scan_blocks(int64_t l);
uint32_t site_scan_block_positions();
void launch_site_scan_slots(hipStream_t st, const uint8_t *refview, int64_t l, SegTab seg, WalkParams wp, int32_t *slots, uint32_t slot_cap, uint32_t *aux, int32_t *out, uint32_t cap, uint64_t *n_out, uint32_t *over);
void launch_mark_dirty(hipStream_t st, const Event *ev, Count n, const int32_t *lo, uint32_t *dirty);
void launch_dirty_chunks(hipStream_t st, bool restore, const uint32_t *dirty, uint32_t n_words, int64_t l_live, const uint8_t *ref, const uint8_t *refview, const uint16_t *refsumm, const uint16_t *refsumm2,
                         uint8_t *cells0, uint8_t *cells1, uint8_t *view0, uint8_t *view1, uint16_t *summ0, uint16_t *summ1, uint16_t *summ2_0, uint16_t *summ2_1);
void launch_scan_excl(hipStream_t st, uint32_t *data, uint32_t n, uint64_t *total_out);
void launch_compact(hipStream_t st, const uint16_t *mask, const uint32_t *block_base, int32_t *out, int64_t l, uint32_t cap);
void launch_events(hipStream_t st, const int32_t *cand, Count n, const uint8_t *ref, SegTab seg, WalkParams wp, Event *ev, uint32_t *max_del);
void walk_debug_seg_min(uint32_t rows);
void launch_resolve(hipStream_t st, Event *ev, Count n, const uint32_t *max_del, uint4 *flags, uint32_t *tot4);
void launch_apply(hipStream_t st, Event *ev, Count n, const uint4 *flags, ContigDev c, WalkParams wp);
void launch_justify_seq(hipStream_t st, const Event *ev, Count n, ContigDev c);
void launch_justify(hipStream_t st, const Event *ev, Count n, ContigDev c, int32_t *lo, int32_t *sufmin, uint8_t *bound);
void launch_mut_debug(hipStream_t st, const uint8_t *ref, const uint8_t *h0, const uint8_t *h1, int64_t l, uint64_t *verdict);
void launch_make_view(hipStream_t st, const uint8_t *cells0, const uint8_t *cells1, int64_t n_cells, int64_t l_live, uint8_t *view0, uint8_t *view1, uint16_t *summ0, uint16_t *summ1, uint16_t *summ2_0, uint16_t *summ2_1);
void launch_apply_patches(hipStream_t st, const int32_t *pos, const uint16_t *cells, uint32_t n, uint8_t *h0, uint8_t *h1);
void launch_collect_mask(hipStream_t st, const uint8_t *h0, const uint8_t *h1, int64_t l, uint16_t *mask, uint32_t *block_count);
void launch_gather(hipStream_t st, const int32_t *pos, uint32_t n, const uint8_t *ref, const uint8_t *h0, const uint8_t *h1, uint32_t *cells);
void launch_hap_len(hipStream_t st, HapDev h, SegTab seg, int64_t l, uint32_t *block_count);
void launch_hap_write(hipStream_t st, HapDev h, SegTab seg, int64_t l, const uint32_t *block_base, const HapRec *rec, uint32_t n_rec, const uint8_t *pool, uint32_t width, uint8_t *text);
void launch_hapchain_count(hipStream_t st, HapDev h, SegTab seg, int64_t l, uint32_t *block_count);
void launch_hapchain_write(hipStream_t st, HapDev h, SegTab seg, int64_t l, const uint32_t *block_base, ChainEnt *out, uint32_t cap);
void launch_place(hipStream_t st, const SimArgs &a);
bool launch_simulate(hipStream_t st, const SimArgs &a, const SimForm &f);
void launch_truth(hipStream_t st, const SimArgs &a, const TruthArgs &t, const DepthArgs *depth);
void launch_truth_depth(hipStream_t st, const SimArgs &a, const TruthArgs &t, const DepthArgs &depth);
int sim_instances(int64_t *out, int cap);
void launch_calibrate(hipStream_t st, const CalibArgs &a);
void launch_failrule(hipStream_t st, const uint32_t *meta, uint64_t n_pairs, uint32_t opens_contig, uint64_t *summ, uint64_t *counters, uint64_t *chain);
void launch_chain_set(hipStream_t st, uint64_t *chain, uint64_t rand_base, int set_rand, uint64_t carry, int set_carry);
void launch_init(hipStream_t st, uint64_t *counters, uint32_t n_counters, uint64_t *z0, uint64_t n0, uint64_t *z1, uint64_t n1, uint64_t *chain, uint64_t rand_base, int set_rand, uint64_t carry, int set_carry);
void launch_selftest_lazy(hipStream_t st, int mode, uint32_t first, uint64_t n, double sigma, float qk, float qeps, float qlmin, int qnear1, uint64_t *out);
uint64_t gz_chunks(uint64_t n);
uint64_t gz_capacity(uint64_t n);
void gz_host_tables(uint32_t *crc_table, uint32_t *crc_shift);
void launch_gzip(hipStream_t st, const uint8_t *text, const uint64_t *n_dev, uint64_t text_cap, uint8_t *out, uint64_t out_cap, uint64_t *status, uint64_t *ticket, uint64_t *total, uint64_t *flags,
                 const uint32_t *crc_table, const uint32_t *crc_shift);
void launch_count_byte(hipStream_t st, const uint8_t *text, uint64_t n, uint32_t byte, uint64_t *out);
void launch_selftest_fp64(hipStream_t st, uint32_t seed, uint64_t n, uint64_t *mism);
void launch_selftest_text(hipStream_t st, uint64_t first, uint64_t n, uint64_t stride, uint64_t *out);
void launch_selftest_gap(hipStream_t st, const uint32_t *lg, uint64_t R, int sR, uint32_t first, uint64_t n, uint32_t g_lo, uint32_t g_cnt, uint32_t *chg, uint64_t *out);
}
```

dwgsim_amd/csrc/dw_walk.hip:

```cpp
#include "dw_device.hpp"
#include "dw_launch.hpp"
#include <stdlib.h>

namespace dw {

__global__ void k_pack(const uint8_t *__restrict__ ascii, uint8_t *__restrict__ ref, uint8_t *__restrict__ h0,
                       uint8_t *__restrict__ h1, int64_t l)
{
    const int64_t nchunk = (l + 15) >> 4;
    for (int64_t ch = (int64_t)blockIdx.x * blockDim.x + threadIdx.x; ch < nchunk; ch += (int64_t)gridDim.x * blockDim.x) {
        const int64_t p0 = ch << 4;
        uint32_t w[4] = {0, 0, 0, 0};
        if (p0 + 16 <= l) {
            const uint4 v = *reinterpret_cast<const uint4 *>(ascii + p0);
            const uint32_t in[4] = {v.x, v.y, v.z, v.w};
#pragma unroll
            for (int q = 0; q < 4; ++q)
#pragma unroll
                for (int b = 0; b < 4; ++b) w[q] |= code_of_ascii((in[q] >> (8 * b)) & 0xff) << (8 * b);
        } else {
            for (int b = 0; b < 16; ++b) { const uint32_t c = (p0 + b < l) ? code_of_ascii(ascii[p0 + b]) : 4u; w[b >> 2] |= c << (8 * (b & 3)); }
        }
        const uint4 o = make_uint4(w[0], w[1], w[2], w[3]);
        *reinterpret_cast<uint4 *>(ref + p0) = o;
        *reinterpret_cast<uint4 *>(h0 + p0) = o;
        *reinterpret_cast<uint4 *>(h1 + p0) = o;
    }
}

constexpr int SITE_WINDOW = 256, SITE_THREADS = 256, SITE_BLOCK_POS = SITE_WINDOW * SITE_THREADS;
static_assert(GROUP_ALIGN % SITE_WINDOW == 0, "a window lies inside one contig: contigs start at multiples of GROUP_ALIGN");
struct SiteChain {
    uint32_t m, w0, w1, w2, w3;
    DW_DEV uint32_t gap(RngKey key, uint32_t q, const WalkParams &wp, const uint32_t *lg)
    {
        if ((m & 3u) == 0u) { const U4 b = rng_block<false>(key, D_WALK_SITE, (uint64_t)q, 0, 0, m >> 2); w0 = b.x; w1 = b.y; w2 = b.z; w3 = b.w; }
        const uint32_t k = m & 3u; ++m;
        const uint32_t w = (k & 2u) ? ((k & 1u) ? w3 : w2) : ((k & 1u) ? w1 : w0);
        return wp.mut_thr >= 0x100000000ull ? 0u : geom_gap(w, lg, wp.gap_r, wp.gap_s);
    }
};
template <class F>
DW_DEV uint32_t site_window(const uint8_t *__restrict__ refview, int64_t l_total, const SegTab &seg, const WalkParams &wp, const uint32_t *lg, int64_t g0, F &&f)
{
    if (g0 >= l_total || wp.mut_thr == 0) return 0;
    const uint32_t sk = seg_of(seg, g0);
    const int64_t p0 = g0 - seg.start[sk], l = seg.len[sk];
    if (p0 >= l) return 0;
    const RngKey key{wp.seed, seg.cindex[sk]};
    const uint32_t q = (uint32_t)(p0 >> 8);
    const uint32_t lim = l - p0 < SITE_WINDOW ? (uint32_t)(l - p0) : (uint32_t)SITE_WINDOW;
    SiteChain ch; ch.m = 0; ch.w0 = ch.w1 = ch.w2 = ch.w3 = 0;
    uint32_t n = 0;
    for (uint32_t S = ch.gap(key, q, wp, lg); S < lim; S += 1u + ch.gap(key, q, wp, lg)) {
        const int64_t g = g0 + S;
        const uint32_t nib = (refview[g >> 1] >> (4 * (g & 1))) & 15u;
        if (nib < 4u) { f(g, n); ++n; }
    }
    return n;
}

__global__ void __launch_bounds__(SITE_THREADS) k_site_scan_list(const uint8_t *__restrict__ refview, int64_t l_total, SegTab seg, WalkParams wp, uint64_t *status, uint64_t *ticket,
                                                              int32_t *__restrict__ out, uint32_t cap, uint64_t *n_out, uint32_t n_blocks)
{
    __shared__ uint32_t sm[1][16], s_lg[FLOW_LG_ENTRIES];
    __shared__ uint32_t s_t; __shared__ uint64_t s_base;
    for (int q = (int)threadIdx.x; q < FLOW_LG_ENTRIES; q += SITE_THREADS) s_lg[q] = wp.lg[q];
    if (threadIdx.x == 0) s_t = (uint32_t)atomicAdd((unsigned long long *)ticket, 1ull);
    __syncthreads();
    const uint32_t t = uniform_u32(s_t);
    const int64_t g0 = ((int64_t)t * SITE_THREADS + threadIdx.x) * SITE_WINDOW;
    const uint32_t cnt[1] = {site_window(refview, l_total, seg, wp, s_lg, g0, [](int64_t, uint32_t) {})};
    uint32_t off[1], tot[1];
    block_excl_scan_n<1>(cnt, sm, off, tot);
    if (threadIdx.x < 64) {
        const uint64_t g = lookback_excl(status, t, tot[0], 0);
        if (threadIdx.x == 0) { s_base = g; if (t + 1 == n_blocks) *n_out = g + tot[0]; }
    }
    __syncthreads();
    const uint64_t at0 = s_base + off[0];
    if (cnt[0]) (void)site_window(refview, l_total, seg, wp, s_lg, g0, [&](int64_t g, uint32_t k) { if (at0 + k < cap) out[at0 + k] = (int32_t)g; });
}

__global__ void __launch_bounds__(SITE_THREADS) k_site_scan_slots(const uint8_t *__restrict__ refview, int64_t l_total, SegTab seg, WalkParams wp, int32_t *__restrict__ slots, uint32_t slot_cap,
                                                               uint32_t *__restrict__ slot_cnt)
{
    __shared__ uint32_t sm[1][16], s_lg[FLOW_LG_ENTRIES];
    for (int q = (int)threadIdx.x; q < FLOW_LG_ENTRIES; q += SITE_THREADS) s_lg[q] = wp.lg[q];
    __syncthreads();
    const uint32_t t = blockIdx.x;
    const int64_t g0 = ((int64_t)t * SITE_THREADS + threadIdx.x) * SITE_WINDOW;
    const uint32_t cnt[1] = {site_window(refview, l_total, seg, wp, s_lg, g0, [](int64_t, uint32_t) {})};
    uint32_t off[1], tot[1];
    block_excl_scan_n<1>(cnt, sm, off, tot);
    if (threadIdx.x == 0) slot_cnt[t] = tot[0];
    int32_t *const slot = slots + (size_t)t * slot_cap;
    const uint32_t at0 = off[0];
    if (cnt[0]) (void)site_window(refview, l_total, seg, wp, s_lg, g0, [&](int64_t g, uint32_t k) { if (at0 + k < slot_cap) slot[at0 + k] = (int32_t)g; });
}
__global__ void __launch_bounds__(1024) k_slot_scan(const uint32_t *__restrict__ slot_cnt, uint32_t nb, uint32_t slot_cap, uint32_t *__restrict__ slot_base, uint64_t *n_out, uint32_t *over)
{
    __shared__ uint32_t sm[17];
    __shared__ uint32_t s_over;
    if (threadIdx.x == 0) s_over = 0;
    const uint32_t per = (nb + 1023u) / 1024u, a = threadIdx.x * per, b = a + per < nb ? a + per : nb;
    uint32_t sum = 0; bool big = false;
    for (uint32_t q = a; q < b; ++q) { const uint32_t c = slot_cnt[q]; sum += c; big |= c > slot_cap; }
    uint32_t total;
    uint32_t run = block_excl_scan(sum, sm, &total);
    if (big) atomicOr(&s_over, 1u);
    for (uint32_t q = a; q < b; ++q) { slot_base[q] = run; run += slot_cnt[q]; }
    __syncthreads();
    if (threadIdx.x == 0) { const bool o = s_over != 0; *n_out = o ? 0ull : (uint64_t)total; if (o) { over[0] = 1u; over[1] = total; } }
}
__global__ void __launch_bounds__(256) k_slot_gather(const int32_t *__restrict__ slots, uint32_t slot_cap, const uint32_t *__restrict__ slot_cnt, const uint32_t *__restrict__ slot_base,
                                                     int32_t *__restrict__ out, uint32_t cap)
{
    const uint32_t t = blockIdx.x, base = slot_base[t];
    uint32_t n = slot_cnt[t]; if (n > slot_cap) n = slot_cap;
    for (uint32_t k = threadIdx.x; k < n; k += 256u) if (base + k < cap) out[base + k] = slots[(size_t)t * slot_cap + k];
}

__global__ void k_mark_dirty(const Event *__restrict__ ev, Count nc, const int32_t *__restrict__ lo, uint32_t *__restrict__ dirty)
{
    const uint32_t n = count_of(nc), k = blockIdx.x * blockDim.x + threadIdx.x;
    if (k >= n) return;
    const Event e = ev[k];
    if (!e.live) return;
    const int64_t right = (int64_t)e.pos + (e.type == 2 ? (int64_t)e.len - 1 : 0);
    const int64_t a = (int64_t)(lo[k] < e.pos ? lo[k] : e.pos) >> 6, b = right >> 6;
    for (int64_t q = a; q <= b; ++q) atomicOr(&dirty[q >> 5], 1u << (q & 31));
}
template <bool RESTORE, bool PER_CHUNK>
__global__ void __launch_bounds__(256) k_dirty_chunks(const uint32_t *__restrict__ dirty, uint32_t n_words, int64_t l_live, const uint8_t *__restrict__ ref, const uint8_t *__restrict__ refview,
                                                      const uint16_t *__restrict__ refsumm, const uint16_t *__restrict__ refsumm2,
                                                      uint8_t *__restrict__ cells0, uint8_t *__restrict__ cells1, uint8_t *__restrict__ view0, uint8_t *__restrict__ view1,
                                                      uint16_t *__restrict__ summ0, uint16_t *__restrict__ summ1, uint16_t *__restrict__ summ2_0, uint16_t *__restrict__ summ2_1)
{
    const uint64_t gid = (uint64_t)blockIdx.x * 256u + threadIdx.x;
    const uint32_t w = PER_CHUNK ? (uint32_t)(gid >> 5) : (uint32_t)gid;
    const bool in = w < n_words;
    const uint32_t touched = in ? dirty[w] : 0u;
    if (PER_CHUNK) { if (!__ballot(touched != 0u)) return; }
    else if (!touched) return;
    uint32_t bits = PER_CHUNK ? ((touched >> (gid & 31u)) & 1u) << (gid & 31u) : touched;
    uint32_t fine[2] = {0u, 0u};
    const bool mine = bits != 0u;
    while (bits) {
        const int q = __ffs((int)bits) - 1; bits &= bits - 1;
        const int64_t ch = (int64_t)w * 32 + q, first = ch * SUMM_CELLS;
        if (RESTORE) {
#pragma unroll
            for (int k = 0; k < SUMM_CELLS / 16; ++k) { const uint4 v = *reinterpret_cast<const uint4 *>(ref + first + 16 * k); *reinterpret_cast<uint4 *>(cells0 + first + 16 * k) = v; *reinterpret_cast<uint4 *>(cells1 + first + 16 * k) = v; }
#pragma unroll
            for (int k = 0; k < SUMM_CELLS / 32; ++k) { const uint4 v = *reinterpret_cast<const uint4 *>(refview + (first >> 1) + 16 * k); *reinterpret_cast<uint4 *>(view0 + (first >> 1) + 16 * k) = v; *reinterpret_cast<uint4 *>(view1 + (first >> 1) + 16 * k) = v; }
            const uint16_t sv = refsumm[ch]; summ0[ch] = sv; summ1[ch] = sv;
        } else {
#pragma unroll
            for (int h = 0; h < 2; ++h) {
                const uint8_t *cells = h ? cells1 : cells0; uint8_t *view = h ? view1 : view0;
                uint32_t indel = 0, non_acgt = 0;
#pragma unroll
                for (int half = 0; half < SUMM_CELLS / 32; ++half) {
                    uint32_t out[4] = {0, 0, 0, 0};
#pragma unroll
                    for (int qq = 0; qq < 2; ++qq) {
                        const int64_t at = first + 32 * half + 16 * qq;
                        const uint4 v = *reinterpret_cast<const uint4 *>(cells + at);
                        const uint32_t wd[4] = {v.x, v.y, v.z, v.w};
#pragma unroll
                        for (int b = 0; b < 16; ++b) {
                            const uint32_t c = (wd[b >> 2] >> (8 * (b & 3))) & 0xffu, ty = c & TMASK, base = c & 0xfu;
                            const uint32_t nib = ty == T_NONE ? (base < 4 ? base : base == 4 ? 8u : 9u) : (ty == T_SUB && base < 4) ? 4u + base : 15u;
                            const int cell = 16 * qq + b;
                            out[cell >> 3] |= nib << (4 * (cell & 7));
                        }
#pragma unroll
                        for (int k = 0; k < 4; ++k) {
                            const int64_t rem = l_live - (at + 4 * k);
                            const uint32_t lm = rem >= 4 ? 0xFFFFFFFFu : rem <= 0 ? 0u : ((1u << (8 * (int)rem)) - 1u);
                            indel += (uint32_t)__popc(wd[k] & lm & 0x10101010u);
                            non_acgt |= wd[k] & lm & 0x0C0C0C0Cu;
                        }
                    }
                    *reinterpret_cast<uint4 *>(view + ((first + 32 * half) >> 1)) = make_uint4(out[0], out[1], out[2], out[3]);
                }
                fine[h] = indel | (non_acgt ? 0x8000u : 0u);
                (h ? summ1 : summ0)[ch] = (uint16_t)fine[h];
            }
        }
    }
    static_assert(SUMM2_CELLS / SUMM_CELLS == 16, "a coarse summary = the sixteen lanes of half a bitmap word");
    if (!PER_CHUNK) {
#pragma unroll
        for (int half = 0; half < 2; ++half) {
            if (!((touched >> (16 * half)) & 0xFFFFu)) continue;
            const int64_t s2 = (int64_t)w * 2 + half;
            if (s2 * SUMM2_CELLS >= l_live) continue;
            if (RESTORE) { const uint16_t sv = refsumm2[s2]; summ2_0[s2] = sv; summ2_1[s2] = sv; }
            else {
#pragma unroll
                for (int h = 0; h < 2; ++h) {
                    const uint16_t *sm1 = h ? summ1 : summ0;
                    uint32_t cnt = 0, fl = 0;
                    for (int k = 0; k < SUMM2_CELLS / SUMM_CELLS; ++k) { const int64_t c2 = s2 * (SUMM2_CELLS / SUMM_CELLS) + k; if (c2 * SUMM_CELLS < l_live) { const uint32_t v = sm1[c2]; cnt += v & 0x7fffu; fl |= v & 0x8000u; } }
                    (h ? summ2_1 : summ2_0)[s2] = (uint16_t)(cnt | fl);
                }
            }
        }
        return;
    }
    const int q = (int)(gid & 31u);
    const int64_t ch = (int64_t)w * 32 + q;
    const int64_t s2 = (int64_t)w * 2 + (q >> 4);
    const bool live2 = in && ((touched >> (16 * (q >> 4))) & 0xFFFFu) != 0u && s2 * SUMM2_CELLS < l_live;
    if (RESTORE) { if (live2 && (q & 15) == 0) { const uint16_t sv = refsumm2[s2]; summ2_0[s2] = sv; summ2_1[s2] = sv; } }
    else {
#pragma unroll
        for (int h = 0; h < 2; ++h) {
            uint32_t v = 0;
            if (live2 && ch * SUMM_CELLS < l_live) v = mine ? fine[h] : (uint32_t)(h ? summ1 : summ0)[ch];
            uint32_t cnt = v & 0x7fffu, fl = v & 0x8000u;
#pragma unroll
            for (int m = 1; m < 16; m <<= 1) { cnt += (uint32_t)__shfl_xor((int)cnt, m); fl |= (uint32_t)__shfl_xor((int)fl, m); }
            if (live2 && (q & 15) == 0) (h ? summ2_1 : summ2_0)[s2] = (uint16_t)(cnt | fl);
        }
    }
}

__global__ void k_scan_excl(uint32_t *data, uint32_t n, uint64_t *total_out)
{
    __shared__ uint32_t sm[2][1][16];
    uint64_t grand = 0; int buf = 0;
    for (uint32_t base = 0; base < n; base += blockDim.x, buf ^= 1) {
        const uint32_t i = base + threadIdx.x;
        const uint32_t v[1] = {i < n ? data[i] : 0u};
        uint32_t ex[1], total[1];
        block_excl_scan_n<1>(v, sm[buf], ex, total);
        if (i < n) data[i] = ex[0] + (uint32_t)grand;
        grand += total[0];
    }
    if (total_out && threadIdx.x == 0) *total_out = grand;
}

__global__ void k_compact(const uint16_t *__restrict__ mask, const uint32_t *__restrict__ block_base, int32_t *__restrict__ out, uint32_t cap)
{
    __shared__ uint32_t sm[17];
    uint32_t bits = mask[(int64_t)blockIdx.x * SCAN_THREADS + threadIdx.x];
    uint32_t total;
    uint32_t off = block_base[blockIdx.x] + block_excl_scan((uint32_t)__popc(bits), sm, &total);
    const int64_t p0 = ((int64_t)blockIdx.x * SCAN_THREADS + threadIdx.x) * SCAN_POS_PER_THREAD;
    while (bits) { const int b = __ffs((int)bits) - 1; bits &= bits - 1; if (off < cap) out[off] = (int32_t)(p0 + b); ++off; }
}

__global__ void k_events(const int32_t *__restrict__ cand, Count nc, const uint8_t *__restrict__ ref, SegTab seg,
                         WalkParams wp, Event *__restrict__ ev, uint32_t *__restrict__ max_del)
{
    const uint32_t n_cand = count_of(nc);
    const uint32_t k = blockIdx.x * blockDim.x + threadIdx.x;
    if (k < n_cand) {
        const int64_t g = cand[k];
        const uint32_t sk = seg_of(seg, g);
        const RngKey key{wp.seed, seg.cindex[sk]};
        const int64_t p = g - seg.start[sk], l = seg.len[sk];
        const uint32_t c = ref[g];
        const U4 b1 = rng_block<false>(key, D_WALK, (uint64_t)p, 0, 0, 1);
        const U4 b2 = rng_block<false>(key, D_WALK, (uint64_t)p, 0, 0, 2);
        Event e; e.pos = (int32_t)g; e.live = 1; e.len = 1; e.base = (uint8_t)c; e.seg = sk;
        if (u_lo(b1) >= wp.indel_frac) {
            e.type = 1;
            e.base = (uint8_t)((c + (uint32_t)(uint64_t)(u_hi(b1) * 3.0 + 1)) & 3);
            e.hap = (wp.is_hap || u_lo(b2) < 0.333333) ? 3 : (u_hi(b2) < 0.5 ? 1 : 2);
        } else if (u_hi(b1) < 0.5) {
            e.type = 2;
            e.hap = (wp.is_hap || u_lo(b2) < 0.3333333) ? 3 : (u_hi(b2) < 0.5 ? 1 : 2);
            uint32_t len = 1;
            for (int64_t q = p + 1; q < l; ++q) {
                if ((int64_t)len < wp.indel_min || rng_slot<false>(key, D_WALK, (uint64_t)q, 0, 0) < wp.indel_extend) ++len; else break;
            }
            e.len = len;
            atomicMax(max_del, len);
        } else {
            e.type = 3;
            uint64_t num = 0; uint32_t kk = 0;
// ... 379 lines not shown
    const int64_t end = (int64_t)seg.start[sk] + seg.len[sk];
    uint32_t cnt = 0;
    if (g < end) { const uint4 v = *reinterpret_cast<const uint4 *>(h.cells + g); cnt = hap_emitted(h, g, v, end - g < 16 ? (int)(end - g) : 16); }
    uint32_t total;
    (void)block_excl_scan(cnt, sm, &total);
    if (threadIdx.x == 0) block_count[blockIdx.x] = total;
}
__global__ void __launch_bounds__(64) k_hap_headers(const HapRec *__restrict__ rec, uint32_t n_rec, const uint8_t *__restrict__ pool, uint8_t *__restrict__ text)
{
    for (uint32_t k = blockIdx.x; k < n_rec; k += gridDim.x) {
        const HapRec R = rec[k];
        for (uint32_t i = threadIdx.x; i < R.hdr_len; i += blockDim.x) text[R.rec_off + i] = pool[R.hdr_off + i];
    }
}
__global__ void __launch_bounds__(SCAN_THREADS) k_hap_write(HapDev h, SegTab seg, const uint32_t *__restrict__ block_base, const HapRec *__restrict__ rec, uint32_t width, uint8_t *__restrict__ text)
{
    __shared__ uint32_t sm[17];
    __shared__ uint32_t s_txt[HAP_WINDOW / 4];
    uint8_t *const stage = reinterpret_cast<uint8_t *>(s_txt);
    const int64_t g0 = (int64_t)blockIdx.x * SCAN_POS_PER_BLOCK, g = g0 + (int64_t)threadIdx.x * SCAN_POS_PER_THREAD;
    const uint32_t sk = seg_of(seg, g0);
    const int64_t end = (int64_t)seg.start[sk] + seg.len[sk];
    uint4 v = make_uint4(0, 0, 0, 0); int nv = 0; uint32_t cnt = 0;
    if (g < end) { v = *reinterpret_cast<const uint4 *>(h.cells + g); nv = end - g < 16 ? (int)(end - g) : 16; cnt = hap_emitted(h, g, v, nv); }
    uint32_t total;
    const uint32_t off = block_excl_scan(cnt, sm, &total);
    if (total == 0) return;
    const HapRec R = rec[sk];
    const uint32_t B = block_base[blockIdx.x] - R.base0, len = R.n_bases;
    const uint64_t body = R.rec_off + R.hdr_len;
    const uint64_t body_bytes = (uint64_t)len + (width ? ((uint64_t)len + width - 1) / width : 1u);
    const bool plain = ((v.x | v.y | v.z | v.w) & 0x10101010u) == 0;
    for (uint32_t w0 = 0; w0 < total; w0 += HAP_WINDOW) {
        const uint32_t nb = total - w0 < (uint32_t)HAP_WINDOW ? total - w0 : (uint32_t)HAP_WINDOW;
        if (w0) __syncthreads();
        if (cnt && off < w0 + nb && off + cnt > w0) {
            uint32_t e = off;
            auto put = [&](uint32_t code) { if (e >= w0 && e - w0 < nb) stage[e - w0] = (uint8_t)hap_char(code); ++e; };
            for (int q = 0; q < nv; ++q) {
                const uint32_t c = hap_cell(v, q), ty = c & TMASK;
                if (ty == T_DEL) continue;
                put(c & 0xfu);
                if (!plain && ty == T_INS) {
                    const uint32_t idx = hap_ins_entry(h, g + q);
                    if (idx < h.n_ins) { const uint32_t n = h.ins_len[idx]; const uint8_t *P = h.ins_bases + h.ins_off[idx]; for (uint32_t j = 0; j < n; ++j) put(P[j]); }
                }
            }
        }
        __syncthreads();
        const uint32_t b0 = B + w0, b1 = b0 + nb;
        const uint32_t r0 = width ? b0 % width : 0u;
        const uint64_t aS = body + b0 + (width ? b0 / width : 0u);
        const uint64_t aE = body + (b1 == len ? body_bytes : (uint64_t)b1 + (width ? b1 / width : 0u));
        for (uint64_t wa = (aS & ~(uint64_t)15) + 16u * (uint64_t)threadIdx.x; wa < aE; wa += 16u * (uint64_t)SCAN_THREADS) {
            const int first = wa < aS ? (int)(aS - wa) : 0;
            const uint32_t d = (uint32_t)(wa + (uint64_t)first - aS), x = r0 + d;
            uint32_t line = 0, col = x;
            if (width) { line = x / (width + 1u); col = x - line * (width + 1u); }
            uint32_t bl = line * width + col - r0;
            uint32_t out[4] = {0, 0, 0, 0};
#pragma unroll
            for (int i = 0; i < 16; ++i) {
                if (i < first || wa + (uint64_t)i >= aE) continue;
                const bool nl = width && col == width;
                const uint32_t ch = (nl || bl >= nb) ? (uint32_t)'\n' : (uint32_t)stage[bl];
                if (nl) col = 0; else { ++col; ++bl; }
                out[i >> 2] |= ch << (8 * (i & 3));
            }
            if (first == 0 && wa + 16u <= aE) *reinterpret_cast<uint4 *>(text + wa) = make_uint4(out[0], out[1], out[2], out[3]);
            else {
#pragma unroll
                for (int i = 0; i < 16; ++i) if (i >= first && wa + (uint64_t)i < aE) text[wa + (uint64_t)i] = (uint8_t)(out[i >> 2] >> (8 * (i & 3)));
            }
        }
    }
}

DW_DEV uint32_t hapchain_ins(const HapDev &h, int64_t g, uint32_t cell)
{
    if ((cell & TMASK) != T_INS) return 0;
    const uint32_t idx = hap_ins_entry(h, g);
    return idx < h.n_ins ? h.ins_len[idx] : 0u;
}
template <class Emit>
DW_DEV uint32_t hapchain_entries(const HapDev &h, int64_t g, const uint4 &v, int nv, int64_t start, int64_t end, Emit emit)
{
    const bool first = g == start, last = g + nv == end;
    const uint32_t pb = first ? 0u : (uint32_t)h.cells[g - 1], nb = last ? 0u : (uint32_t)h.cells[g + nv];
    if (!first && !last && (((v.x | v.y | v.z | v.w) | pb | nb) & 0x10101010u) == 0) return 0;
    uint32_t n = 0;
    bool gap = first || (pb & TMASK) == T_DEL || hapchain_ins(h, g - 1, pb) > 0;
    for (int q = 0; q < nv; ++q) {
        const uint32_t c = hap_cell(v, q);
        if ((c & TMASK) == T_DEL) { gap = true; continue; }
        const uint32_t ins = hapchain_ins(h, g + q, c);
        const bool more = q + 1 < nv || !last;
        const uint32_t nx = q + 1 < nv ? hap_cell(v, q + 1) : nb;
        if (gap) { emit((uint32_t)(g + q - start), 0u); ++n; }
        if (ins > 0 || !more || (nx & TMASK) == T_DEL) { emit((uint32_t)(g + q - start), CHAIN_END | ins); ++n; }
        gap = ins > 0;
    }
    return n;
}
__global__ void __launch_bounds__(SCAN_THREADS) k_hapchain_count(HapDev h, SegTab seg, uint32_t *__restrict__ block_count)
{
    __shared__ uint32_t sm[17];
    const int64_t g0 = (int64_t)blockIdx.x * SCAN_POS_PER_BLOCK, g = g0 + (int64_t)threadIdx.x * SCAN_POS_PER_THREAD;
    const uint32_t sk = seg_of(seg, g0);
    const int64_t start = (int64_t)seg.start[sk], end = start + seg.len[sk];
    uint32_t cnt = 0;
    if (g < end) { const uint4 v = *reinterpret_cast<const uint4 *>(h.cells + g); cnt = hapchain_entries(h, g, v, end - g < 16 ? (int)(end - g) : 16, start, end, [](uint32_t, uint32_t) {}); }
    uint32_t total;
    (void)block_excl_scan(cnt, sm, &total);
    if (threadIdx.x == 0) block_count[blockIdx.x] = total;
}
__global__ void __launch_bounds__(SCAN_THREADS) k_hapchain_write(HapDev h, SegTab seg, const uint32_t *__restrict__ block_base, ChainEnt *__restrict__ out, uint32_t cap)
{
    __shared__ uint32_t sm[17];
    const int64_t g0 = (int64_t)blockIdx.x * SCAN_POS_PER_BLOCK, g = g0 + (int64_t)threadIdx.x * SCAN_POS_PER_THREAD;
    const uint32_t sk = seg_of(seg, g0);
    const int64_t start = (int64_t)seg.start[sk], end = start + seg.len[sk];
    uint4 v = make_uint4(0, 0, 0, 0); int nv = 0; uint32_t cnt = 0;
    if (g < end) { v = *reinterpret_cast<const uint4 *>(h.cells + g); nv = end - g < 16 ? (int)(end - g) : 16; cnt = hapchain_entries(h, g, v, nv, start, end, [](uint32_t, uint32_t) {}); }
    uint32_t total;
    const uint32_t off = block_excl_scan(cnt, sm, &total);
    if (cnt == 0) return;
    uint32_t at = block_base[blockIdx.x] + off;
    (void)hapchain_entries(h, g, v, nv, start, end, [&](uint32_t pos, uint32_t info) { if (at < cap) out[at] = ChainEnt{pos, info}; ++at; });
}

void launch_hapchain_count(hipStream_t st, HapDev h, SegTab seg, int64_t l, uint32_t *block_count)
{
    if (l > 0) hipLaunchKernelGGL(k_hapchain_count, dim3(cdiv((uint64_t)l, SCAN_POS_PER_BLOCK)), dim3(SCAN_THREADS), 0, st, h, seg, block_count);
}
void launch_hapchain_write(hipStream_t st, HapDev h, SegTab seg, int64_t l, const uint32_t *block_base, ChainEnt *out, uint32_t cap)
{
    if (l > 0 && cap > 0) hipLaunchKernelGGL(k_hapchain_write, dim3(cdiv((uint64_t)l, SCAN_POS_PER_BLOCK)), dim3(SCAN_THREADS), 0, st, h, seg, block_base, out, cap);
}
void launch_hap_len(hipStream_t st, HapDev h, SegTab seg, int64_t l, uint32_t *block_count)
{
    if (l > 0) hipLaunchKernelGGL(k_hap_len, dim3(cdiv((uint64_t)l, SCAN_POS_PER_BLOCK)), dim3(SCAN_THREADS), 0, st, h, seg, block_count);
}
void launch_hap_write(hipStream_t st, HapDev h, SegTab seg, int64_t l, const uint32_t *block_base, const HapRec *rec, uint32_t n_rec, const uint8_t *pool, uint32_t width, uint8_t *text)
{
    if (n_rec) hipLaunchKernelGGL(k_hap_headers, dim3(n_rec < 4096u ? n_rec : 4096u), dim3(64), 0, st, rec, n_rec, pool, text);
    if (l > 0) hipLaunchKernelGGL(k_hap_write, dim3(cdiv((uint64_t)l, SCAN_POS_PER_BLOCK)), dim3(SCAN_THREADS), 0, st, h, seg, block_base, rec, width, text);
}
void launch_pack(hipStream_t st, const uint8_t *ascii, uint8_t *ref, uint8_t *h0, uint8_t *h1, int64_t l)
{
    const uint64_t nchunk = (uint64_t)(l + 15) >> 4;
    uint32_t nb = cdiv(nchunk, 256); if (nb > (1u << 16)) nb = 1u << 16; if (nb == 0) nb = 1;
    hipLaunchKernelGGL(k_pack, dim3(nb), dim3(256), 0, st, ascii, ref, h0, h1, l);
}
void launch_site_scan_list(hipStream_t st, const uint8_t *refview, int64_t l, SegTab seg, WalkParams wp, uint64_t *status, uint64_t *ticket, int32_t *out, uint32_t cap, uint64_t *n_out)
{
    const uint32_t nb = (uint32_t)cdiv((uint64_t)l, (uint64_t)SITE_BLOCK_POS);
    hipLaunchKernelGGL(k_site_scan_list, dim3(nb), dim3(SITE_THREADS), 0, st, refview, l, seg, wp, status, ticket, out, cap, n_out, nb);
}
uint32_t site_scan_blocks(int64_t l) { return (uint32_t)cdiv((uint64_t)l, (uint64_t)SITE_BLOCK_POS); }
uint32_t site_scan_block_positions() { return (uint32_t)SITE_BLOCK_POS; }
void launch_site_scan_slots(hipStream_t st, const uint8_t *refview, int64_t l, SegTab seg, WalkParams wp, int32_t *slots, uint32_t slot_cap, uint32_t *aux, int32_t *out, uint32_t cap, uint64_t *n_out, uint32_t *over)
{
    const uint32_t nb = site_scan_blocks(l);
    if (!nb) return;
    hipLaunchKernelGGL(k_site_scan_slots, dim3(nb), dim3(SITE_THREADS), 0, st, refview, l, seg, wp, slots, slot_cap, aux);
    hipLaunchKernelGGL(k_slot_scan, dim3(1), dim3(1024), 0, st, aux, nb, slot_cap, aux + nb, n_out, over);
    hipLaunchKernelGGL(k_slot_gather, dim3(nb), dim3(256), 0, st, slots, slot_cap, aux, aux + nb, out, cap);
}
void launch_mark_dirty(hipStream_t st, const Event *ev, Count n, const int32_t *lo, uint32_t *dirty)
{
    if (n.host) hipLaunchKernelGGL(k_mark_dirty, dim3(cdiv(n.host, 256)), dim3(256), 0, st, ev, n, lo, dirty);
}
void launch_dirty_chunks(hipStream_t st, bool restore, const uint32_t *dirty, uint32_t n_words, int64_t l_live, const uint8_t *ref, const uint8_t *refview, const uint16_t *refsumm, const uint16_t *refsumm2,
                         uint8_t *cells0, uint8_t *cells1, uint8_t *view0, uint8_t *view1, uint16_t *summ0, uint16_t *summ1, uint16_t *summ2_0, uint16_t *summ2_1)
{
    if (!n_words) return;
    bool per_chunk = (uint64_t)n_words * 32 <= (1ull << 21);
    if (const char *e = getenv("DWGSIM_HIP_DIRTY_MAP")) per_chunk = e[0] == 'c';
    const dim3 grid(cdiv((uint64_t)n_words * (per_chunk ? 32 : 1), 256));
    if (restore) { if (per_chunk) hipLaunchKernelGGL((k_dirty_chunks<true, true>), grid, dim3(256), 0, st, dirty, n_words, l_live, ref, refview, refsumm, refsumm2, cells0, cells1, view0, view1, summ0, summ1, summ2_0, summ2_1); else hipLaunchKernelGGL((k_dirty_chunks<true, false>), grid, dim3(256), 0, st, dirty, n_words, l_live, ref, refview, refsumm, refsumm2, cells0, cells1, view0, view1, summ0, summ1, summ2_0, summ2_1); }
    else { if (per_chunk) hipLaunchKernelGGL((k_dirty_chunks<false, true>), grid, dim3(256), 0, st, dirty, n_words, l_live, ref, refview, refsumm, refsumm2, cells0, cells1, view0, view1, summ0, summ1, summ2_0, summ2_1); else hipLaunchKernelGGL((k_dirty_chunks<false, false>), grid, dim3(256), 0, st, dirty, n_words, l_live, ref, refview, refsumm, refsumm2, cells0, cells1, view0, view1, summ0, summ1, summ2_0, summ2_1); }
}
void launch_scan_excl(hipStream_t st, uint32_t *data, uint32_t n, uint64_t *total_out)
{
    hipLaunchKernelGGL(k_scan_excl, dim3(1), dim3(1024), 0, st, data, n, total_out);
}
void launch_compact(hipStream_t st, const uint16_t *mask, const uint32_t *block_base, int32_t *out, int64_t l, uint32_t cap)
{
    hipLaunchKernelGGL(k_compact, dim3(cdiv((uint64_t)l, SCAN_POS_PER_BLOCK)), dim3(SCAN_THREADS), 0, st, mask, block_base, out, cap);
}
void launch_events(hipStream_t st, const int32_t *cand, Count n, const uint8_t *ref, SegTab seg, WalkParams wp, Event *ev, uint32_t *max_del)
{
    if (n.host) hipLaunchKernelGGL(k_events, dim3(cdiv(n.host, 256)), dim3(256), 0, st, cand, n, ref, seg, wp, ev, max_del);
}
void launch_resolve(hipStream_t st, Event *ev, Count n, const uint32_t *max_del, uint4 *flags, uint32_t *tot4)
{
    if (n.host) hipLaunchKernelGGL(k_resolve, dim3(cdiv(n.host, 256)), dim3(256), 0, st, ev, n, max_del, flags);
    if (n.host < g_walk_seg_min_rows) { hipLaunchKernelGGL(k_scan4, dim3(1), dim3(1024), 0, st, flags, n, tot4, 0u, (uint4 *)nullptr); return; }
    const uint32_t seglen = (n.host + WALK_SEGS - 1) / WALK_SEGS;
    hipLaunchKernelGGL(k_scan4, dim3(WALK_SEGS), dim3(1024), 0, st, flags, n, tot4, seglen, flags + n.host);
    hipLaunchKernelGGL(k_scan4_fix, dim3(cdiv(n.host, 256)), dim3(256), 0, st, flags, n, tot4, seglen, (const uint4 *)(flags + n.host));
}
void launch_apply(hipStream_t st, Event *ev, Count n, const uint4 *flags, ContigDev c, WalkParams wp)
{
    if (n.host) hipLaunchKernelGGL(k_apply, dim3(cdiv(n.host, 256)), dim3(256), 0, st, ev, n, flags, c, wp);
}
void launch_justify_seq(hipStream_t st, const Event *ev, Count n, ContigDev c)
{
    if (n.host) hipLaunchKernelGGL(k_justify_seq, dim3(1), dim3(64), 0, st, ev, n, c);
}
void launch_justify(hipStream_t st, const Event *ev, Count n, ContigDev c, int32_t *lo, int32_t *sufmin, uint8_t *bound)
{
    if (!n.host) return;
    hipLaunchKernelGGL(k_jreach, dim3(cdiv(n.host, 256)), dim3(256), 0, st, ev, n, c, lo);
    if (n.host < g_walk_seg_min_rows) hipLaunchKernelGGL(k_sufmin, dim3(1), dim3(1024), 0, st, lo, n, sufmin, 0u, (int32_t *)nullptr);
    else {
        const uint32_t seglen = (n.host + WALK_SEGS - 1) / WALK_SEGS;
        hipLaunchKernelGGL(k_sufmin, dim3(WALK_SEGS), dim3(1024), 0, st, lo, n, sufmin, seglen, sufmin + n.host);
        hipLaunchKernelGGL(k_sufmin_fix, dim3(cdiv(n.host, 256)), dim3(256), 0, st, sufmin, n, seglen, (const int32_t *)(sufmin + n.host));
    }
    hipLaunchKernelGGL(k_jbound, dim3(cdiv(n.host, 256)), dim3(256), 0, st, ev, n, c, sufmin, bound);
    hipLaunchKernelGGL(k_jrun, dim3(cdiv(n.host, 64)), dim3(64), 0, st, ev, n, c, bound);
}
__global__ void __launch_bounds__(SCAN_THREADS) k_mut_debug(const uint8_t *__restrict__ ref, const uint8_t *__restrict__ h0, const uint8_t *__restrict__ h1, int64_t l, uint64_t *verdict)
{
    const int64_t first = ((int64_t)blockIdx.x * SCAN_THREADS + threadIdx.x) * SCAN_POS_PER_THREAD;
    if (first >= l) return;
    const uint4 a = *reinterpret_cast<const uint4 *>(h0 + first), b = *reinterpret_cast<const uint4 *>(h1 + first);
    if ((((a.x | a.y | a.z | a.w) | (b.x | b.y | b.z | b.w)) & 0x30303030u) == 0) return;
    const uint4 r = *reinterpret_cast<const uint4 *>(ref + first);
    const uint32_t aw[4] = {a.x, a.y, a.z, a.w}, bw[4] = {b.x, b.y, b.z, b.w}, rw[4] = {r.x, r.y, r.z, r.w};
    for (int q = 0; q < SCAN_POS_PER_THREAD && first + q < l; ++q) {
        const uint32_t c0 = (rw[q >> 2] >> (8 * (q & 3))) & 0xffu, c1 = (aw[q >> 2] >> (8 * (q & 3))) & 0xffu, c2 = (bw[q >> 2] >> (8 * (q & 3))) & 0xffu;
        if (c0 >= 4 || ((c1 & TMASK) == T_NONE && (c2 & TMASK) == T_NONE)) continue;
        uint32_t code = 0;
        if ((c1 & BTMASK) == (c2 & BTMASK)) { if ((c1 & TMASK) == T_SUB && (c0 & 3) == (c1 & 3)) code = 1; }
        else if ((c1 & TMASK) == T_SUB || (c2 & TMASK) == T_SUB) {
            if ((c1 & 3) == (c2 & 3)) code = 2;
            else if (!((c0 & 3) == (c1 & 3) || (c0 & 3) == (c2 & 3))) code = 3;
        }
        if (code) { atomicMin((unsigned long long *)verdict, ((unsigned long long)(first + q) << 8) | code); return; }
    }
}
void launch_mut_debug(hipStream_t st, const uint8_t *ref, const uint8_t *h0, const uint8_t *h1, int64_t l, uint64_t *verdict)
{
    if (l > 0) hipLaunchKernelGGL(k_mut_debug, dim3(cdiv((uint64_t)l, SCAN_POS_PER_BLOCK)), dim3(SCAN_THREADS), 0, st, ref, h0, h1, l, verdict);
}
__global__ void __launch_bounds__(256) k_make_view(const uint8_t *__restrict__ cells0, const uint8_t *__restrict__ cells1, int64_t n_cells, int64_t l_live, uint8_t *__restrict__ view0, uint8_t *__restrict__ view1,
                                                   uint16_t *__restrict__ summ0, uint16_t *__restrict__ summ1, uint16_t *__restrict__ summ2_0, uint16_t *__restrict__ summ2_1)
{
    const uint8_t *__restrict__ cells = blockIdx.y ? cells1 : cells0;
    uint8_t *__restrict__ view = blockIdx.y ? view1 : view0;
    uint16_t *__restrict__ summ = blockIdx.y ? summ1 : summ0, *__restrict__ summ2 = blockIdx.y ? summ2_1 : summ2_0;
    const int64_t t = (int64_t)blockIdx.x * 256 + threadIdx.x, first = t * 32;
    const bool live = first < n_cells;
    uint32_t out[4] = {0, 0, 0, 0}, indel = 0, non_acgt = 0;
    if (live) {
#pragma unroll
        for (int q = 0; q < 2; ++q) {
            if (first + 16 * q >= n_cells) break;
            const uint4 v = *reinterpret_cast<const uint4 *>(cells + first + 16 * q);
            const uint32_t w[4] = {v.x, v.y, v.z, v.w};
#pragma unroll
            for (int b = 0; b < 16; ++b) {
                const uint32_t c = (w[b >> 2] >> (8 * (b & 3))) & 0xffu, ty = c & TMASK, base = c & 0xfu;
                const uint32_t nib = ty == T_NONE ? (base < 4 ? base : base == 4 ? 8u : 9u) : (ty == T_SUB && base < 4) ? 4u + base : 15u;
                const int cell = 16 * q + b;
                out[cell >> 3] |= nib << (4 * (cell & 7));
            }
#pragma unroll
            for (int k = 0; k < 4; ++k) {
                const int64_t rem = l_live - (first + 16 * q + 4 * k);
                const uint32_t lm = rem >= 4 ? 0xFFFFFFFFu : rem <= 0 ? 0u : ((1u << (8 * (int)rem)) - 1u);
                indel += (uint32_t)__popc(w[k] & lm & 0x10101010u);
                non_acgt |= w[k] & lm & 0x0C0C0C0Cu;
            }
        }
        *reinterpret_cast<uint4 *>(view + (first >> 1)) = make_uint4(out[0], out[1], out[2], out[3]);
    }
    uint32_t i1 = indel, f1 = non_acgt ? 1u : 0u;
#pragma unroll
    for (int d = 1; d < SUMM_CELLS / 32; d <<= 1) { i1 += (uint32_t)__shfl_xor((int)i1, d); f1 |= (uint32_t)__shfl_xor((int)f1, d); }
    uint32_t i2 = i1, f2 = f1;
#pragma unroll
    for (int d = SUMM_CELLS / 32; d < SUMM2_CELLS / 32; d <<= 1) { i2 += (uint32_t)__shfl_xor((int)i2, d); f2 |= (uint32_t)__shfl_xor((int)f2, d); }
    if (first < l_live) {
        if ((t & (SUMM_CELLS / 32 - 1)) == 0) summ[t / (SUMM_CELLS / 32)] = (uint16_t)(i1 | (f1 ? 0x8000u : 0u));
        if ((t & (SUMM2_CELLS / 32 - 1)) == 0) summ2[t / (SUMM2_CELLS / 32)] = (uint16_t)(i2 | (f2 ? 0x8000u : 0u));
    }
}
void launch_make_view(hipStream_t st, const uint8_t *cells0, const uint8_t *cells1, int64_t n_cells, int64_t l_live, uint8_t *view0, uint8_t *view1, uint16_t *summ0, uint16_t *summ1, uint16_t *summ2_0, uint16_t *summ2_1)
{
    if (n_cells > 0) hipLaunchKernelGGL(k_make_view, dim3(cdiv((uint64_t)n_cells, 256 * 32), 2), dim3(256), 0, st, cells0, cells1, n_cells, l_live, view0, view1, summ0, summ1, summ2_0, summ2_1);
}
void launch_apply_patches(hipStream_t st, const int32_t *pos, const uint16_t *cells, uint32_t n, uint8_t *h0, uint8_t *h1)
{
    if (n) hipLaunchKernelGGL(k_apply_patches, dim3(cdiv(n, 256)), dim3(256), 0, st, pos, cells, n, h0, h1);
}
void launch_collect_mask(hipStream_t st, const uint8_t *h0, const uint8_t *h1, int64_t l, uint16_t *mask, uint32_t *block_count)
{
    hipLaunchKernelGGL(k_collect_mask, dim3(cdiv((uint64_t)l, SCAN_POS_PER_BLOCK)), dim3(SCAN_THREADS), 0, st, h0, h1, l, mask, block_count);
}
void launch_gather(hipStream_t st, const int32_t *pos, uint32_t n, const uint8_t *ref, const uint8_t *h0, const uint8_t *h1, uint32_t *cells)
{
    if (n) hipLaunchKernelGGL(k_gather, dim3(cdiv(n, 256)), dim3(256), 0, st, pos, n, ref, h0, h1, cells);
}

}
```

Before: 1525.

## Track dirty chunks in a compact list instead of scanning the full bitmap

Mark-dirty now also appends each newly dirtied chunk index to a device list. View and summary rebuild and restore kernels then visit only the listed chunks instead of scanning every bitmap word. Restore clears bits atomically, so the memset of the dirty map is skipped. Counter zeroing moves into the site-scan kernel, replacing a separate memset. If the list overflows, the code falls back to the bitmap path with an extra host sync, and it adds atomics and extra debug hooks.

Result: faster. 1555 (median of 6 runs) (+2.0%).

```diff
diff --git a/dwgsim_amd/csrc/dw_host.cpp b/dwgsim_amd/csrc/dw_host.cpp
--- a/dwgsim_amd/csrc/dw_host.cpp
+++ b/dwgsim_amd/csrc/dw_host.cpp
@@ -45,6 +45,7 @@
     std::vector<uint8_t> h_names; std::vector<int32_t> h_reg, h_seg;
     DevMem d_summ[2], d_summ2[2];
     DevMem d_refview, d_refsumm, d_refsumm2, d_dirty;
+    DevMem d_dlist;
     DevEvent ev_walk, ev_walk0;
     DevMem d_hap_text[2], d_hap_rec, d_hap_pool;
     DevMem d_hap_chain[2];
@@ -57,7 +58,7 @@
     uint64_t n_cand;
     uint32_t max_del;
     struct { uint32_t entries, bases; } ins[2];
-    uint32_t unused1;
+    uint32_t list_over;
     uint32_t slot_over;
     uint32_t n_cand_true;
     uint64_t mut_debug[2];
@@ -69,6 +70,8 @@
               offsetof(WalkCounters, n_cand_true) == 8 * 8 + 7 * 4 && offsetof(WalkCounters, mut_debug) == 12 * 8 && offsetof(WalkCounters, n_listed) == 14 * 8, "every counter at the word the kernels were given before the block had a type");
 struct WcSpan { size_t off, bytes; };
 #define WC_SPAN(first, last) WcSpan{offsetof(WalkCounters, first), offsetof(WalkCounters, last) + sizeof(WalkCounters::last) - offsetof(WalkCounters, first)}
+constexpr WcSpan WC_ZEROED = WC_SPAN(max_del, n_cand_true);
+static_assert(offsetof(WalkCounters, max_del) == offsetof(WalkCounters, n_cand) + sizeof(uint64_t) && WC_ZEROED.bytes % sizeof(uint32_t) == 0, "WC_RANDOM = n_cand, then the words that are cleared");
 constexpr WcSpan WC_RANDOM = WC_SPAN(n_cand, n_cand_true), WC_FILE = WC_SPAN(mut_debug, mut_debug), WC_LISTED = WC_SPAN(n_listed, n_listed);
 
 struct Group {
@@ -81,6 +84,7 @@
     int fixed_max = 0;
     uint32_t n_cand = 0;
     bool dirty_any = false, dirty_all = false;
+    uint32_t dirty_listed = 0;
     int walk_attempt = 0; uint32_t walk_cap = 0; size_t walk_cap_bases = 0; bool walk_reset = false;
     uint32_t n_patch = 0, n_patch_ev = 0;
     bool list_valid = false; std::vector<int32_t> pos; std::vector<uint32_t> cells; HostIns ins[2];
@@ -138,6 +142,9 @@
         uint64_t place_open = 0; double walk_us = 0, count_us = 0;
         int64_t sim_form = 0;
         int64_t walk_form = 0;
+        int dirty_list = -1; int64_t dirty_list_cap = -1;
+        int64_t state_hash = 0;
+        int64_t dirty_list_walks = 0, dirty_list_restores = 0, dirty_fallbacks = 0;
         double hap_len_us = 0, hap_write_us = 0, hap_copy_us = 0, truth_us = 0, truth_copy_us = 0; bool hap_yardstick = false; double chain_count_us = 0, chain_write_us = 0; int64_t chain_blocks = 0;
     } dbg;
     int device = 0;
@@ -254,9 +261,9 @@
 
 size_t view_bytes(size_t padded) { return padded / 2; }
 size_t summ_bytes(size_t padded) { return sizeof(uint16_t) * (padded / SUMM_CELLS); }
-size_t summ2_bytes(size_t padded) { return sizeof(uint16_t) * (padded / SUMM2_CELLS); }
+size_t summ2_bytes(size_t padded) { return sizeof(uint16_t) * ((padded + SUMM2_CELLS - 1) / SUMM2_CELLS); }
 uint32_t dirty_words(size_t padded) { return (uint32_t)((padded + 32 * SUMM_CELLS - 1) / (32 * SUMM_CELLS)); }
-size_t dirty_bytes(size_t padded) { return sizeof(uint32_t) * ((size_t)dirty_words(padded) + 2); }
+size_t dirty_bytes(size_t padded) { return sizeof(uint32_t) * ((size_t)dirty_words(padded) + 3); }
 
 enum : unsigned { R_CELLS = 1, R_VIEW = 2, R_SUMM = 4, R_SUMM2 = 8, R_ALL = 15 };
 int restore_pristine(dwgsim_hip_ctx *c, const Group &g, int h, unsigned what, hipStream_t st)
@@ -274,6 +281,12 @@
 {
     HIPC(c, hipMemsetAsync(g.mem.d_dirty.get(), 0, dirty_bytes(padded_cells(g)), st));
     return 0;
+}
+
+uint32_t *dirty_count(const Group &g) { return g.mem.d_dirty.get<uint32_t>() + dirty_words(padded_cells(g)) + 2; }
+DirtyList dirty_list(dwgsim_hip_ctx *c, const Group &g, uint32_t cap)
+{
+    return DirtyList{cap ? g.mem.d_dlist.get<uint32_t>() : nullptr, dirty_count(g), cap, &c->d_wcounters.get<WalkCounters>()->list_over};
 }
 
 hipError_t wc_fill(dwgsim_hip_ctx *c, WcSpan s, int byte, hipStream_t st) { return hipMemsetAsync(c->d_wcounters.get() + s.off, byte, s.bytes, st); }
@@ -976,6 +989,12 @@
     launch_dirty_chunks(st, restore, M.d_dirty.get<uint32_t>(), dirty_words(padded_cells(g)), g.total, M.d_ref.get(), M.d_refview.get(), M.d_refsumm.get<uint16_t>(), M.d_refsumm2.get<uint16_t>(),
                         M.d_cells[0].get(), M.d_cells[1].get(), M.d_view[0].get(), M.d_view[1].get(), M.d_summ[0].get<uint16_t>(), M.d_summ[1].get<uint16_t>(), M.d_summ2[0].get<uint16_t>(), M.d_summ2[1].get<uint16_t>());
 }
+static void listed_chunks(hipStream_t st, bool restore, const Group &g, DirtyList list)
+{
+    const GroupMem &M = g.mem;
+    launch_list_chunks(st, restore, list, M.d_dirty.get<uint32_t>(), g.total, M.d_ref.get(), M.d_refview.get(), M.d_refsumm.get<uint16_t>(), M.d_refsumm2.get<uint16_t>(),
+                       M.d_cells[0].get(), M.d_cells[1].get(), M.d_view[0].get(), M.d_view[1].get(), M.d_summ[0].get<uint16_t>(), M.d_summ[1].get<uint16_t>(), M.d_summ2[0].get<uint16_t>(), M.d_summ2[1].get<uint16_t>());
+}
 
 static void justify(dwgsim_hip_ctx_t *c, hipStream_t st, const Event *ev, Count n, const ContigDev &cd)
 {
@@ -1025,6 +1044,8 @@
     bool use_slots; uint32_t nbs, slot_cap; size_t slot_bytes;
     Restore restore;
     bool dense;
+    uint32_t list_cap;
+    uint32_t list_restore;
 };
 
 static WalkPlan walk_plan(const dwgsim_hip_ctx_t *c, const Group &g)
@@ -1040,6 +1061,10 @@
     P.use_slots = g.walk_attempt == 0 && c->dbg.site_slots != 0 && P.nbs > 0 && (c->dbg.site_slots > 0 || P.slot_bytes <= std::max<size_t>((size_t)64 << 20, P.ncap * 16));
     P.restore = g.walk_attempt > 0 || g.dirty_all ? Restore::All : g.dirty_any ? Restore::Chunks : Restore::None;
     P.dense = c->dbg.seq_justify || c->dbg.dense_view;
+    const uint64_t n_chunks = (uint64_t)dirty_words(padded_cells(g)) * 32;
+    P.list_cap = P.dense || c->dbg.dirty_list == 0 || dirty_map_forced() ? 0u : (uint32_t)std::min<uint64_t>(n_chunks, 2 * (uint64_t)P.cap + 64);
+    if (P.list_cap && c->dbg.dirty_list_cap > 0) P.list_cap = (uint32_t)std::min<uint64_t>(n_chunks, (uint64_t)c->dbg.dirty_list_cap);
+    P.list_restore = P.restore == Restore::Chunks && g.mem.d_dlist.cap() >= sizeof(uint32_t) * (size_t)P.list_cap ? g.dirty_listed : 0u;
     return P;
 }
 
@@ -1052,6 +1077,7 @@
         ensure(c, c->w_bound, P.ncap)) return DWGSIM_HIP_ERR_DEVICE;
     for (int h = 0; h < 2; ++h) if (const int rc = ensure_ins(c, g, h, P.ncap, P.cap_bases)) return rc;
     if (P.use_slots && (ensure(c, c->w_slots, P.slot_bytes) || ensure(c, c->w_slot_aux, 2 * (size_t)P.nbs * sizeof(uint32_t)))) return DWGSIM_HIP_ERR_DEVICE;
+    if (P.list_cap && ensure(c, g.mem.d_dlist, sizeof(uint32_t) * (size_t)P.list_cap)) return DWGSIM_HIP_ERR_DEVICE;
     return DWGSIM_HIP_OK;
 }
 
@@ -1065,12 +1091,12 @@
     int32_t *d_cand = c->w_cand.get<int32_t>(); Event *d_ev = c->w_ev.get<Event>(); uint4 *d_flags = c->w_flags.get<uint4>();
     uint32_t *tot4 = &wc->ins[0].entries;
     const Count nc{&wc->n_cand, P.cap};
-    HIPC(c, wc_fill(c, WC_RANDOM, 0, st));
-    if (P.use_slots) launch_site_scan_slots(st, M.d_refview.get(), g.total, seg, wp, c->w_slots.get<int32_t>(), P.slot_cap, c->w_slot_aux.get<uint32_t>(), d_cand, P.cap, &wc->n_cand, &wc->slot_over);
+    const WalkZero zero{&wc->max_del, (uint32_t)(WC_ZEROED.bytes / sizeof(uint32_t)), dirty_count(g)};
+    if (P.use_slots) launch_site_scan_slots(st, M.d_refview.get(), g.total, seg, wp, c->w_slots.get<int32_t>(), P.slot_cap, c->w_slot_aux.get<uint32_t>(), d_cand, P.cap, &wc->n_cand, &wc->slot_over, zero);
     else {
         uint64_t *d_status = c->scratch_status.get<uint64_t>();
         HIPC(c, hipMemsetAsync(d_status, 0, ((size_t)P.nblk + 2) * sizeof(uint64_t), st));
-        launch_site_scan_list(st, M.d_refview.get(), g.total, seg, wp, d_status, d_status + P.nblk, d_cand, P.cap, &wc->n_cand);
+        launch_site_scan_list(st, M.d_refview.get(), g.total, seg, wp, d_status, d_status + P.nblk, d_cand, P.cap, &wc->n_cand, zero);
     }
     launch_events(st, d_cand, nc, M.d_ref.get(), seg, wp, d_ev, &wc->max_del);
     launch_resolve(st, d_ev, nc, &wc->max_del, d_flags, tot4);
@@ -1082,9 +1108,11 @@
         make_views(st, g);
         g.dirty_all = true;
     } else {
-        launch_mark_dirty(st, d_ev, nc, c->w_lo.get<int32_t>(), M.d_dirty.get<uint32_t>());
-        dirty_chunks(st, false, g);
-        g.dirty_any = true;
+        const DirtyList list = dirty_list(c, g, P.list_cap);
+        launch_mark_dirty(st, d_ev, nc, c->w_lo.get<int32_t>(), M.d_dirty.get<uint32_t>(), list);
+        if (P.list_cap) { listed_chunks(st, false, g, list); ++c->dbg.dirty_list_walks; }
+        else dirty_chunks(st, false, g);
+        g.dirty_any = true; g.dirty_listed = P.list_cap;
     }
     HIPC(c, hipGetLastError());
     return DWGSIM_HIP_OK;
@@ -1098,8 +1126,9 @@
     hipStream_t st = c->walk_stream.get();
     HIPC(c, hipEventRecord(g.mem.ev_walk0.get(), st));
     if (P.restore == Restore::All) { for (int h = 0; h < 2; ++h) if (const int rc = restore_pristine(c, g, h, R_ALL, st)) return rc; }
+    else if (P.list_restore) { listed_chunks(st, true, g, dirty_list(c, g, P.list_restore)); ++c->dbg.dirty_list_restores; }
     else if (P.restore == Restore::Chunks) dirty_chunks(st, true, g);
-    if (P.restore != Restore::None) { if (const int rc = clear_dirty(c, g, st)) return rc; g.dirty_all = g.dirty_any = false; }
+    if (P.restore != Restore::None) { if (!P.list_restore) { if (const int rc = clear_dirty(c, g, st)) return rc; } g.dirty_all = g.dirty_any = false; g.dirty_listed = 0; }
     if (const int rc = walk_launch(c, g, P)) return rc;
     HIPC(c, wc_fetch(c, g.mem, WC_RANDOM, st));
     HIPC(c, hipEventRecord(g.mem.ev_walk.get(), st));
@@ -1200,6 +1229,13 @@
         if (fits || g.walk_attempt >= 2) {
             g.walk_pending = false;
             if (!fits) { c->err = "mutation walk: capacities still exceeded after an exact re-run"; return DWGSIM_HIP_ERR_FAILED; }
+            if (g.dirty_listed && w.list_over) {
+                g.dirty_listed = 0; ++c->dbg.dirty_fallbacks;
+                dirty_chunks(c->walk_stream.get(), false, g);
+                HIPC(c, hipGetLastError());
+                HIPC(c, hipEventRecord(g.mem.ev_walk.get(), c->walk_stream.get()));
+                HIPC(c, hipEventSynchronize(g.mem.ev_walk.get()));
+            }
             g.n_cand = (uint32_t)w.n_cand;
             for (int h = 0; h < 2; ++h) { g.n_ins[h] = w.ins[h].entries; g.n_ins_bases[h] = w.ins[h].bases; }
             return DWGSIM_HIP_OK;
@@ -2428,6 +2464,26 @@
     else if (!strcmp(key, "walk_cap")) c->dbg.walk_cap = value;
     else if (!strcmp(key, "site_slots")) c->dbg.site_slots = (int)value;
     else if (!strcmp(key, "site_slot_cap")) c->dbg.site_slot_cap = value;
+    else if (!strcmp(key, "dirty_list")) c->dbg.dirty_list = (int)value;
+    else if (!strcmp(key, "dirty_list_cap")) c->dbg.dirty_list_cap = value;
+    else if (!strcmp(key, "state_hash")) {
+        const Group *g = get_group(c, (int)value);
+        if (!g || !g->mutated || g->walk_pending) { c->err = "state_hash: no finished walk of that contig's group"; return DWGSIM_HIP_ERR_ARG; }
+        HIPC(c, hipSetDevice(c->device));
+        HIPC(c, hipStreamSynchronize(c->walk_stream.get()));
+        const size_t n1 = ((size_t)g->total + SUMM_CELLS - 1) / SUMM_CELLS, n2 = ((size_t)g->total + SUMM2_CELLS - 1) / SUMM2_CELLS;
+        std::vector<uint8_t> host;
+        uint64_t x = 0xcbf29ce484222325ull;
+        for (int h = 0; h < 2; ++h) {
+            const struct { const DevMem &buf; size_t bytes; } parts[] = {{g->mem.d_view[h], (size_t)g->total / 2}, {g->mem.d_summ[h], sizeof(uint16_t) * n1}, {g->mem.d_summ2[h], sizeof(uint16_t) * n2}};
+            for (const auto &part : parts) {
+                host.resize(part.bytes);
+                if (part.bytes) HIPC(c, hipMemcpy(host.data(), part.buf.get(), part.bytes, hipMemcpyDeviceToHost));
+                for (const uint8_t b : host) x = (x ^ b) * 0x100000001b3ull;
+            }
+        }
+        c->dbg.state_hash = (int64_t)x;
+    }
     else if (!strcmp(key, "phases")) c->dbg.phases = value != 0;
     else if (!strcmp(key, "writer")) c->dbg.writer = (int)value;
     else if (!strcmp(key, "sim_threads")) c->dbg.force_threads = (int)value;
@@ -2474,6 +2530,10 @@
     else if (!strcmp(key, "truth_us")) *value = (int64_t)c->dbg.truth_us;
     else if (!strcmp(key, "truth_reruns")) *value = c->dbg.truth_reruns;
     else if (!strcmp(key, "truth_copy_us")) *value = (int64_t)c->dbg.truth_copy_us;
+    else if (!strcmp(key, "state_hash")) *value = c->dbg.state_hash;
+    else if (!strcmp(key, "dirty_list_walks")) *value = c->dbg.dirty_list_walks;
+    else if (!strcmp(key, "dirty_list_restores")) *value = c->dbg.dirty_list_restores;
+    else if (!strcmp(key, "dirty_fallbacks")) *value = c->dbg.dirty_fallbacks;
     else if (!strcmp(key, "walk_form")) *value = c->dbg.walk_form;
     else { c->err = "unknown debug value"; return DWGSIM_HIP_ERR_ARG; }
     return DWGSIM_HIP_OK;
diff --git a/dwgsim_amd/csrc/dw_kernels.hpp b/dwgsim_amd/csrc/dw_kernels.hpp
--- a/dwgsim_amd/csrc/dw_kernels.hpp
+++ b/dwgsim_amd/csrc/dw_kernels.hpp
@@ -77,6 +77,9 @@
 constexpr int HAP_WINDOW = 8192;
 
 struct Count { const uint64_t *dev; uint32_t host; };
+
+struct DirtyList { uint32_t *idx; uint32_t *count; uint32_t cap; uint32_t *over; };
+struct WalkZero { uint32_t *wc; uint32_t n_wc; uint32_t *list_count; };
 
 struct WalkParams {
     double mut_rate, indel_frac, indel_extend;
diff --git a/dwgsim_amd/csrc/dw_launch.hpp b/dwgsim_amd/csrc/dw_launch.hpp
--- a/dwgsim_amd/csrc/dw_launch.hpp
+++ b/dwgsim_amd/csrc/dw_launch.hpp
@@ -4,11 +4,14 @@
 
 namespace dw {
 void launch_pack(hipStream_t st, const uint8_t *ascii, uint8_t *ref, uint8_t *h0, uint8_t *h1, int64_t l);
-void launch_site_scan_list(hipStream_t st, const uint8_t *refview, int64_t l, SegTab seg, WalkParams wp, uint64_t *status, uint64_t *ticket, int32_t *out, uint32_t cap, uint64_t *n_out);
+void launch_site_scan_list(hipStream_t st, const uint8_t *refview, int64_t l, SegTab seg, WalkParams wp, uint64_t *status, uint64_t *ticket, int32_t *out, uint32_t cap, uint64_t *n_out, WalkZero zero);
 uint32_t site_scan_blocks(int64_t l);
 uint32_t site_scan_block_positions();
-void launch_site_scan_slots(hipStream_t st, const uint8_t *refview, int64_t l, SegTab seg, WalkParams wp, int32_t *slots, uint32_t slot_cap, uint32_t *aux, int32_t *out, uint32_t cap, uint64_t *n_out, uint32_t *over);
-void launch_mark_dirty(hipStream_t st, const Event *ev, Count n, const int32_t *lo, uint32_t *dirty);
+void launch_site_scan_slots(hipStream_t st, const uint8_t *refview, int64_t l, SegTab seg, WalkParams wp, int32_t *slots, uint32_t slot_cap, uint32_t *aux, int32_t *out, uint32_t cap, uint64_t *n_out, uint32_t *over, WalkZero zero);
+void launch_mark_dirty(hipStream_t st, const Event *ev, Count n, const int32_t *lo, uint32_t *dirty, DirtyList list);
+bool dirty_map_forced();
+void launch_list_chunks(hipStream_t st, bool restore, DirtyList list, uint32_t *dirty, int64_t l_live, const uint8_t *ref, const uint8_t *refview, const uint16_t *refsumm, const uint16_t *refsumm2,
+                        uint8_t *cells0, uint8_t *cells1, uint8_t *view0, uint8_t *view1, uint16_t *summ0, uint16_t *summ1, uint16_t *summ2_0, uint16_t *summ2_1);
 void launch_dirty_chunks(hipStream_t st, bool restore, const uint32_t *dirty, uint32_t n_words, int64_t l_live, const uint8_t *ref, const uint8_t *refview, const uint16_t *refsumm, const uint16_t *refsumm2,
                          uint8_t *cells0, uint8_t *cells1, uint8_t *view0, uint8_t *view1, uint16_t *summ0, uint16_t *summ1, uint16_t *summ2_0, uint16_t *summ2_1);
 void launch_scan_excl(hipStream_t st, uint32_t *data, uint32_t n, uint64_t *total_out);
diff --git a/dwgsim_amd/csrc/dw_walk.hip b/dwgsim_amd/csrc/dw_walk.hip
--- a/dwgsim_amd/csrc/dw_walk.hip
+++ b/dwgsim_amd/csrc/dw_walk.hip
@@ -60,11 +60,19 @@
     return n;
 }
 
+DW_DEV void walk_zero(const WalkZero &z)
+{
+    if (blockIdx.x != 0) return;
+    if (threadIdx.x < z.n_wc) z.wc[threadIdx.x] = 0u;
+    if (threadIdx.x == 0 && z.list_count) *z.list_count = 0u;
+}
+
 __global__ void __launch_bounds__(SITE_THREADS) k_site_scan_list(const uint8_t *__restrict__ refview, int64_t l_total, SegTab seg, WalkParams wp, uint64_t *status, uint64_t *ticket,
-                                                              int32_t *__restrict__ out, uint32_t cap, uint64_t *n_out, uint32_t n_blocks)
+                                                              int32_t *__restrict__ out, uint32_t cap, uint64_t *n_out, uint32_t n_blocks, WalkZero zero)
 {
     __shared__ uint32_t sm[1][16], s_lg[FLOW_LG_ENTRIES];
     __shared__ uint32_t s_t; __shared__ uint64_t s_base;
+    walk_zero(zero);
     for (int q = (int)threadIdx.x; q < FLOW_LG_ENTRIES; q += SITE_THREADS) s_lg[q] = wp.lg[q];
     if (threadIdx.x == 0) s_t = (uint32_t)atomicAdd((unsigned long long *)ticket, 1ull);
     __syncthreads();
@@ -83,9 +91,10 @@
 }
 
 __global__ void __launch_bounds__(SITE_THREADS) k_site_scan_slots(const uint8_t *__restrict__ refview, int64_t l_total, SegTab seg, WalkParams wp, int32_t *__restrict__ slots, uint32_t slot_cap,
-                                                               uint32_t *__restrict__ slot_cnt)
+                                                               uint32_t *__restrict__ slot_cnt, WalkZero zero)
 {
     __shared__ uint32_t sm[1][16], s_lg[FLOW_LG_ENTRIES];
+    walk_zero(zero);
     for (int q = (int)threadIdx.x; q < FLOW_LG_ENTRIES; q += SITE_THREADS) s_lg[q] = wp.lg[q];
     __syncthreads();
     const uint32_t t = blockIdx.x;
@@ -121,7 +130,7 @@
     for (uint32_t k = threadIdx.x; k < n; k += 256u) if (base + k < cap) out[base + k] = slots[(size_t)t * slot_cap + k];
 }
 
-__global__ void k_mark_dirty(const Event *__restrict__ ev, Count nc, const int32_t *__restrict__ lo, uint32_t *__restrict__ dirty)
+__global__ void k_mark_dirty(const Event *__restrict__ ev, Count nc, const int32_t *__restrict__ lo, uint32_t *__restrict__ dirty, DirtyList list)
 {
     const uint32_t n = count_of(nc), k = blockIdx.x * blockDim.x + threadIdx.x;
     if (k >= n) return;
@@ -129,7 +138,70 @@
     if (!e.live) return;
     const int64_t right = (int64_t)e.pos + (e.type == 2 ? (int64_t)e.len - 1 : 0);
     const int64_t a = (int64_t)(lo[k] < e.pos ? lo[k] : e.pos) >> 6, b = right >> 6;
-    for (int64_t q = a; q <= b; ++q) atomicOr(&dirty[q >> 5], 1u << (q & 31));
+    for (int64_t q = a; q <= b; ++q) {
+        const uint32_t bit = 1u << (q & 31), before = atomicOr(&dirty[q >> 5], bit);
+        if (!list.idx || (before & bit)) continue;
+        const uint32_t at = atomicAdd(list.count, 1u);
+        if (at < list.cap) list.idx[at] = (uint32_t)q; else *list.over = 1u;
+    }
+}
+template <bool RESTORE>
+__global__ void __launch_bounds__(256) k_list_chunks(DirtyList list, uint32_t *__restrict__ dirty, int64_t l_live, const uint8_t *__restrict__ ref, const uint8_t *__restrict__ refview,
+                                                     const uint16_t *__restrict__ refsumm, const uint16_t *__restrict__ refsumm2,
+                                                     uint8_t *__restrict__ cells0, uint8_t *__restrict__ cells1, uint8_t *__restrict__ view0, uint8_t *__restrict__ view1,
+                                                     uint16_t *__restrict__ summ0, uint16_t *__restrict__ summ1, uint16_t *__restrict__ summ2_0, uint16_t *__restrict__ summ2_1)
+{
+    static_assert(SUMM_CELLS == 64 && SUMM2_CELLS / SUMM_CELLS == 16, "sixteen lanes of four cells are a chunk; sixteen chunks are a coarse summary");
+    const uint32_t listed = *list.count, n = listed < list.cap ? listed : list.cap;
+    const uint32_t slot = blockIdx.x * 16u + (threadIdx.x >> 4), lane = threadIdx.x & 15u;
+    const bool live = slot < n;
+    const int64_t ch = live ? (int64_t)list.idx[slot] : 0, first = ch * SUMM_CELLS + 4 * (int64_t)lane;
+    if (RESTORE) {
+        if (!live) return;
+        const uint32_t v = *reinterpret_cast<const uint32_t *>(ref + first);
+        *reinterpret_cast<uint32_t *>(cells0 + first) = v; *reinterpret_cast<uint32_t *>(cells1 + first) = v;
+        const uint16_t vw = *reinterpret_cast<const uint16_t *>(refview + (first >> 1));
+        *reinterpret_cast<uint16_t *>(view0 + (first >> 1)) = vw; *reinterpret_cast<uint16_t *>(view1 + (first >> 1)) = vw;
+        if (lane == 0) { const uint16_t sv = refsumm[ch]; summ0[ch] = sv; summ1[ch] = sv; }
+        if (lane == 1) { const int64_t s2 = ch >> 4; if (s2 * SUMM2_CELLS < l_live) { const uint16_t sv = refsumm2[s2]; summ2_0[s2] = sv; summ2_1[s2] = sv; } }
+        if (lane == 2) atomicAdd(&dirty[ch >> 5], 0u - (1u << (ch & 31)));
+        return;
+    }
+#pragma unroll
+    for (int h = 0; h < 2; ++h) {
+        const uint8_t *cells = h ? cells1 : cells0;
+        const uint32_t wd = live ? *reinterpret_cast<const uint32_t *>(cells + first) : 0u;
+        uint32_t out = 0;
+#pragma unroll
+        for (int b = 0; b < 4; ++b) {
+            const uint32_t c = (wd >> (8 * b)) & 0xffu, ty = c & TMASK, base = c & 0xfu;
+            const uint32_t nib = ty == T_NONE ? (base < 4 ? base : base == 4 ? 8u : 9u) : (ty == T_SUB && base < 4) ? 4u + base : 15u;
+            out |= nib << (4 * b);
+        }
+        if (live) *reinterpret_cast<uint16_t *>((h ? view1 : view0) + (first >> 1)) = (uint16_t)out;
+        const int64_t rem = l_live - first;
+        const uint32_t lm = rem >= 4 ? 0xFFFFFFFFu : rem <= 0 ? 0u : ((1u << (8 * (int)rem)) - 1u);
+        uint32_t indel = (uint32_t)__popc(wd & lm & 0x10101010u), non_acgt = wd & lm & 0x0C0C0C0Cu;
+#pragma unroll
+        for (int m = 1; m < 16; m <<= 1) { indel += (uint32_t)__shfl_xor((int)indel, m); non_acgt |= (uint32_t)__shfl_xor((int)non_acgt, m); }
+        if (live && lane == 0) (h ? summ1 : summ0)[ch] = (uint16_t)(indel | (non_acgt ? 0x8000u : 0u));
+    }
+}
+__global__ void __launch_bounds__(256) k_list_coarse(DirtyList list, int64_t l_live, const uint16_t *__restrict__ summ0, const uint16_t *__restrict__ summ1,
+                                                     uint16_t *__restrict__ summ2_0, uint16_t *__restrict__ summ2_1)
+{
+    const uint32_t listed = *list.count, n = listed < list.cap ? listed : list.cap;
+    const uint32_t slot = blockIdx.x * 16u + (threadIdx.x >> 4), lane = threadIdx.x & 15u;
+    const bool live = slot < n;
+    const int64_t s2 = live ? (int64_t)(list.idx[slot] >> 4) : 0, c2 = s2 * (SUMM2_CELLS / SUMM_CELLS) + lane;
+#pragma unroll
+    for (int h = 0; h < 2; ++h) {
+        const uint32_t v = live && c2 * SUMM_CELLS < l_live ? (uint32_t)(h ? summ1 : summ0)[c2] : 0u;
+        uint32_t cnt = v & 0x7fffu, fl = v & 0x8000u;
+#pragma unroll
+        for (int m = 1; m < 16; m <<= 1) { cnt += (uint32_t)__shfl_xor((int)cnt, m); fl |= (uint32_t)__shfl_xor((int)fl, m); }
+        if (live && lane == 0 && s2 * SUMM2_CELLS < l_live) (h ? summ2_1 : summ2_0)[s2] = (uint16_t)(cnt | fl);
+    }
 }
 template <bool RESTORE, bool PER_CHUNK>
 __global__ void __launch_bounds__(256) k_dirty_chunks(const uint32_t *__restrict__ dirty, uint32_t n_words, int64_t l_live, const uint8_t *__restrict__ ref, const uint8_t *__restrict__ refview,
@@ -815,24 +887,34 @@
     uint32_t nb = cdiv(nchunk, 256); if (nb > (1u << 16)) nb = 1u << 16; if (nb == 0) nb = 1;
     hipLaunchKernelGGL(k_pack, dim3(nb), dim3(256), 0, st, ascii, ref, h0, h1, l);
 }
-void launch_site_scan_list(hipStream_t st, const uint8_t *refview, int64_t l, SegTab seg, WalkParams wp, uint64_t *status, uint64_t *ticket, int32_t *out, uint32_t cap, uint64_t *n_out)
+void launch_site_scan_list(hipStream_t st, const uint8_t *refview, int64_t l, SegTab seg, WalkParams wp, uint64_t *status, uint64_t *ticket, int32_t *out, uint32_t cap, uint64_t *n_out, WalkZero zero)
 {
     const uint32_t nb = (uint32_t)cdiv((uint64_t)l, (uint64_t)SITE_BLOCK_POS);
-    hipLaunchKernelGGL(k_site_scan_list, dim3(nb), dim3(SITE_THREADS), 0, st, refview, l, seg, wp, status, ticket, out, cap, n_out, nb);
+    hipLaunchKernelGGL(k_site_scan_list, dim3(nb), dim3(SITE_THREADS), 0, st, refview, l, seg, wp, status, ticket, out, cap, n_out, nb, zero);
 }
 uint32_t site_scan_blocks(int64_t l) { return (uint32_t)cdiv((uint64_t)l, (uint64_t)SITE_BLOCK_POS); }
 uint32_t site_scan_block_positions() { return (uint32_t)SITE_BLOCK_POS; }
-void launch_site_scan_slots(hipStream_t st, const uint8_t *refview, int64_t l, SegTab seg, WalkParams wp, int32_t *slots, uint32_t slot_cap, uint32_t *aux, int32_t *out, uint32_t cap, uint64_t *n_out, uint32_t *over)
+void launch_site_scan_slots(hipStream_t st, const uint8_t *refview, int64_t l, SegTab seg, WalkParams wp, int32_t *slots, uint32_t slot_cap, uint32_t *aux, int32_t *out, uint32_t cap, uint64_t *n_out, uint32_t *over, WalkZero zero)
 {
     const uint32_t nb = site_scan_blocks(l);
     if (!nb) return;
-    hipLaunchKernelGGL(k_site_scan_slots, dim3(nb), dim3(SITE_THREADS), 0, st, refview, l, seg, wp, slots, slot_cap, aux);
+    hipLaunchKernelGGL(k_site_scan_slots, dim3(nb), dim3(SITE_THREADS), 0, st, refview, l, seg, wp, slots, slot_cap, aux, zero);
     hipLaunchKernelGGL(k_slot_scan, dim3(1), dim3(1024), 0, st, aux, nb, slot_cap, aux + nb, n_out, over);
     hipLaunchKernelGGL(k_slot_gather, dim3(nb), dim3(256), 0, st, slots, slot_cap, aux, aux + nb, out, cap);
 }
-void launch_mark_dirty(hipStream_t st, const Event *ev, Count n, const int32_t *lo, uint32_t *dirty)
-{
-    if (n.host) hipLaunchKernelGGL(k_mark_dirty, dim3(cdiv(n.host, 256)), dim3(256), 0, st, ev, n, lo, dirty);
+void launch_mark_dirty(hipStream_t st, const Event *ev, Count n, const int32_t *lo, uint32_t *dirty, DirtyList list)
+{
+    if (n.host) hipLaunchKernelGGL(k_mark_dirty, dim3(cdiv(n.host, 256)), dim3(256), 0, st, ev, n, lo, dirty, list);
+}
+bool dirty_map_forced() { return getenv("DWGSIM_HIP_DIRTY_MAP") != nullptr; }
+void launch_list_chunks(hipStream_t st, bool restore, DirtyList list, uint32_t *dirty, int64_t l_live, const uint8_t *ref, const uint8_t *refview, const uint16_t *refsumm, const uint16_t *refsumm2,
+                        uint8_t *cells0, uint8_t *cells1, uint8_t *view0, uint8_t *view1, uint16_t *summ0, uint16_t *summ1, uint16_t *summ2_0, uint16_t *summ2_1)
+{
+    if (!list.cap) return;
+    const dim3 grid(cdiv(list.cap, 16));
+    if (restore) { hipLaunchKernelGGL((k_list_chunks<true>), grid, dim3(256), 0, st, list, dirty, l_live, ref, refview, refsumm, refsumm2, cells0, cells1, view0, view1, summ0, summ1, summ2_0, summ2_1); return; }
+    hipLaunchKernelGGL((k_list_chunks<false>), grid, dim3(256), 0, st, list, dirty, l_live, ref, refview, refsumm, refsumm2, cells0, cells1, view0, view1, summ0, summ1, summ2_0, summ2_1);
+    hipLaunchKernelGGL(k_list_coarse, grid, dim3(256), 0, st, list, l_live, summ0, summ1, summ2_0, summ2_1);
 }
 void launch_dirty_chunks(hipStream_t st, bool restore, const uint32_t *dirty, uint32_t n_words, int64_t l_live, const uint8_t *ref, const uint8_t *refview, const uint16_t *refsumm, const uint16_t *refsumm2,
                          uint8_t *cells0, uint8_t *cells1, uint8_t *view0, uint8_t *view1, uint16_t *summ0, uint16_t *summ1, uint16_t *summ2_0, uint16_t *summ2_1)
```
